# kheder-hassoun/Tf-IDF-Distributed-System

Hardware: AMD Instinct MI355X
Metric: docs indexed/sec + queries scored/sec (node) at 1/2/4/8 GPUs; % HBM roofline (higher is better)
Workload: dtype u8/u32 (integer inversion), f32 BM25 with f64 accumulation

## Files before the change

include/tfidf.h:

```cpp
#ifndef TFIDF_H
#define TFIDF_H

#include <stddef.h>
#include <stdint.h>

#ifdef __cplusplus
extern "C" {
#endif

#define TFIDF_OK 0
#define TFIDF_E_INVALID_ARG 1
#define TFIDF_E_HIP 2
#define TFIDF_E_OOM 3
#define TFIDF_E_UNSUPPORTED_INPUT 4
#define TFIDF_E_UNSUPPORTED_QUERY 5
#define TFIDF_E_CAPACITY 6
#define TFIDF_E_STATE 7
#define TFIDF_E_BUFFER 8
#define TFIDF_E_NO_DEVICE 9
#define TFIDF_E_QUERY_SYNTAX 10

#define TFIDF_STATS_SHARD 0
#define TFIDF_STATS_GLOBAL 1

// ... 6 lines not shown
typedef struct tfidf_config {
  float k1;
  float b;
  int32_t stats_mode;
  int32_t device;
  uint32_t vocab_capacity_log2;
  uint32_t max_token_len;
  int32_t inversion;
} tfidf_config;

typedef struct tfidf_index_stats {
  uint64_t num_docs;
  uint64_t doc_count;
  uint64_t sum_ttf;
  uint64_t num_terms;
  uint64_t nnz;
  uint64_t device_bytes;
  uint64_t long_docs;
  uint64_t text_bytes;
  uint64_t term_major;
  uint64_t pack_docs;
  uint64_t pack_retried;
  uint64_t unicode_docs;
  uint64_t long_chunked;
  uint64_t malformed_docs;
  uint64_t hash_seed;
  uint64_t hash_rebuilds;
  uint64_t coalesced_batches;
  uint64_t coalesced_queries;
  uint64_t unit_batches;
  uint64_t unit_count;
  uint64_t fused_queries;
  uint64_t unicode_wave_docs;
  uint64_t dead_docs;
  uint64_t dead_bytes;
  uint64_t compactions;
} tfidf_index_stats;

typedef struct tfidf_commit_timing {
  float ms_total;
  float ms_tokenize;
  float ms_long;
  float ms_df;
  float ms_blockscan;
  float ms_colscan;
  float ms_scatter;
  uint64_t text_bytes;
  uint64_t num_docs;
  uint64_t nnz;
} tfidf_commit_timing;

enum { TFIDF_MIRROR_NONE = 0, TFIDF_MIRROR_DELTA = 1, TFIDF_MIRROR_WHOLE = 2 };
typedef struct tfidf_host_profile {
  double ms_wall;
  double ms_counters;
  double ms_enqueued;
  double ms_synced;
  double ms_published;
  uint32_t stream_syncs;
  uint32_t col_rank_runs;
  uint32_t mirror_dict, mirror_df, mirror_crank;
  uint32_t dict_delta_entries, df_delta_entries;
  uint64_t bytes_dict, bytes_df, bytes_crank;
} tfidf_host_profile;

const char *tfidf_version(void);
const char *tfidf_last_error(void);
int tfidf_config_init(tfidf_config *cfg);

int tfidf_create(const tfidf_config *cfg, tfidf_index **out);
int tfidf_destroy(tfidf_index *ix);

int tfidf_add_docs(tfidf_index *ix, const uint8_t *utf8, const uint64_t *offsets, uint64_t n_docs,
                   const uint8_t *keys, const uint64_t *key_offsets);
int tfidf_clear(tfidf_index *ix);
int tfidf_add_docs_device(tfidf_index *ix, const void *d_utf8, const void *d_offsets, uint64_t n_docs,
                          uint64_t total_bytes);

int tfidf_commit(tfidf_index *ix);
int tfidf_commit_tokenized_docs(const tfidf_index *ix, uint64_t *docs, uint32_t *was_full);
int tfidf_commit_inverted_blocks(const tfidf_index *ix, uint32_t *first_block, uint32_t *n_blocks,
                                 uint32_t *remapped);
int tfidf_commit_inversion_shape(const tfidf_index *ix, uint32_t *slices, uint32_t *scan_parts);
int tfidf_commit_host_profile(const tfidf_index *ix, tfidf_host_profile *out);

int tfidf_delete_docs(tfidf_index *ix, const uint8_t *keys, const uint64_t *key_offsets, uint64_t n_keys,
                      uint64_t *n_deleted);
int tfidf_compact(tfidf_index *ix, uint64_t *bytes_reclaimed, float *ms_device);
int tfidf_set_compact_threshold(tfidf_index *ix, uint32_t dead_pct);
int tfidf_doc_text(tfidf_index *ix, uint64_t doc, uint8_t *buf, uint64_t cap, uint64_t *n_out);
int tfidf_set_hash_attempt(tfidf_index *ix, uint32_t attempt);

int tfidf_save(tfidf_index *ix, const char *path);
int tfidf_load(tfidf_index *ix, const char *path);
int tfidf_get_commit_timing(const tfidf_index *ix, tfidf_commit_timing *out);
int tfidf_stats(const tfidf_index *ix, tfidf_index_stats *out);

int tfidf_search(tfidf_index *ix, const uint8_t *q, uint64_t q_len, uint32_t k, uint32_t *doc_ids,
                 float *scores, uint64_t cap, uint64_t *n_out);
int tfidf_search_coalesced(tfidf_index *ix, const uint8_t *q, uint64_t q_len, uint32_t k, uint32_t *doc_ids,
                           float *scores, uint64_t cap, uint64_t *n_out, uint32_t wait_us);
int tfidf_search_batch(tfidf_index *ix, const uint8_t *q_utf8, const uint64_t *q_offsets, uint32_t n_q,
                       uint32_t k, uint32_t *doc_ids, float *scores, uint32_t *counts);
int tfidf_search_batch_all(tfidf_index *ix, const uint8_t *q_utf8, const uint64_t *q_offsets, uint32_t n_q,
                           uint32_t *doc_ids, float *scores, uint64_t cap, uint64_t *hit_offsets, uint64_t *n_out);
typedef struct tfidf_reader tfidf_reader;
int tfidf_reader_open(tfidf_index *ix, tfidf_reader **out);
int tfidf_reader_close(tfidf_reader *rd);
int tfidf_reader_info(const tfidf_reader *rd, uint64_t *generation, uint64_t *num_docs);
int tfidf_reader_search(tfidf_reader *rd, const uint8_t *q, uint64_t q_len, uint32_t k, uint32_t *doc_ids,
                        float *scores, uint64_t cap, uint64_t *n_out);
int tfidf_reader_search_batch_all(tfidf_reader *rd, const uint8_t *q_utf8, const uint64_t *q_offsets, uint32_t n_q,
                                  uint32_t *doc_ids, float *scores, uint64_t cap, uint64_t *hit_offsets,
                                  uint64_t *n_out);
int tfidf_reader_doc_key(const tfidf_reader *rd, uint64_t doc, uint8_t *buf, uint64_t cap, uint64_t *n_out);
int tfidf_reader_doc_text(const tfidf_reader *rd, uint64_t doc, uint8_t *buf, uint64_t cap, uint64_t *n_out);
int tfidf_reader_doc_keys(const tfidf_reader *rd, uint8_t *buf, uint64_t cap, uint64_t *offsets, uint64_t *n_bytes);
int tfidf_reader_matches(tfidf_reader *rd, const uint8_t *q, uint64_t q_len, const uint32_t *docs, uint64_t n_docs,
                         uint64_t *starts, uint32_t *lens, uint32_t *ordinals, uint64_t cap,
                         uint64_t *match_offsets, uint64_t *n_out, float *ms_device);
int tfidf_reader_snippets(tfidf_reader *rd, const uint8_t *q, uint64_t q_len, const uint32_t *docs, uint64_t n_docs,
                          uint32_t max_bytes, uint8_t *text, uint64_t text_cap, uint64_t *text_offsets,
                          uint64_t *doc_starts, uint64_t *starts, uint32_t *lens, uint32_t *ordinals, uint64_t m_cap,
                          uint64_t *match_offsets, uint64_t *n_text, uint64_t *n_matches, float *ms_device);
int tfidf_matches(tfidf_index *ix, const uint8_t *q, uint64_t q_len, const uint32_t *docs, uint64_t n_docs,
                  uint64_t *starts, uint32_t *lens, uint32_t *ordinals, uint64_t cap, uint64_t *match_offsets,
                  uint64_t *n_out, float *ms_device);
int tfidf_snippets(tfidf_index *ix, const uint8_t *q, uint64_t q_len, const uint32_t *docs, uint64_t n_docs,
                   uint32_t max_bytes, uint8_t *text, uint64_t text_cap, uint64_t *text_offsets, uint64_t *doc_starts,
                   uint64_t *starts, uint32_t *lens, uint32_t *ordinals, uint64_t m_cap, uint64_t *match_offsets,
                   uint64_t *n_text, uint64_t *n_matches, float *ms_device);
int tfidf_query_positive_terms(const uint8_t *q, uint64_t q_len, char *out, uint64_t cap, uint64_t *n_terms,
                               uint64_t *n_bytes);
int tfidf_reader_matches_batch(tfidf_reader *rd, const uint8_t *q_utf8, const uint64_t *q_offsets, uint32_t n_q,
                               const uint32_t *docs, const uint64_t *doc_offsets, uint64_t *starts, uint32_t *lens,
                               uint32_t *ordinals, uint64_t cap, uint64_t *match_offsets, uint64_t *n_out,
                               float *ms_device);
int tfidf_reader_snippets_batch(tfidf_reader *rd, const uint8_t *q_utf8, const uint64_t *q_offsets, uint32_t n_q,
                                const uint32_t *docs, const uint64_t *doc_offsets, uint32_t max_bytes, uint8_t *text,
                                uint64_t text_cap, uint64_t *text_offsets, uint64_t *doc_starts, uint64_t *starts,
                                uint32_t *lens, uint32_t *ordinals, uint64_t m_cap, uint64_t *match_offsets,
                                uint64_t *n_text, uint64_t *n_matches, float *ms_device);
int tfidf_matches_batch(tfidf_index *ix, const uint8_t *q_utf8, const uint64_t *q_offsets, uint32_t n_q,
                        const uint32_t *docs, const uint64_t *doc_offsets, uint64_t *starts, uint32_t *lens,
                        uint32_t *ordinals, uint64_t cap, uint64_t *match_offsets, uint64_t *n_out, float *ms_device);
int tfidf_snippets_batch(tfidf_index *ix, const uint8_t *q_utf8, const uint64_t *q_offsets, uint32_t n_q,
                         const uint32_t *docs, const uint64_t *doc_offsets, uint32_t max_bytes, uint8_t *text,
                         uint64_t text_cap, uint64_t *text_offsets, uint64_t *doc_starts, uint64_t *starts,
                         uint32_t *lens, uint32_t *ordinals, uint64_t m_cap, uint64_t *match_offsets,
                         uint64_t *n_text, uint64_t *n_matches, float *ms_device);
int tfidf_last_highlight_chunks(const tfidf_index *ix, uint64_t *item_chunks, uint64_t *row_chunks);
int tfidf_fuzzy_terms_batch(tfidf_index *ix, const uint8_t *t_utf8, const uint64_t *t_offsets, uint32_t n_terms,
                            uint32_t max_edits, uint32_t prefix_len, uint32_t max_out, uint64_t *cand_offsets,
                            uint64_t *n_within, uint64_t *term_offsets, uint8_t *terms, uint64_t terms_cap,
                            uint32_t *df, uint8_t *dist, uint64_t cand_cap, uint64_t *n_cands,
                            uint64_t *n_term_bytes, float *ms_device);
int tfidf_reader_fuzzy_terms_batch(tfidf_reader *rd, const uint8_t *t_utf8, const uint64_t *t_offsets,
                                   uint32_t n_terms, uint32_t max_edits, uint32_t prefix_len, uint32_t max_out,
                                   uint64_t *cand_offsets, uint64_t *n_within, uint64_t *term_offsets, uint8_t *terms,
                                   uint64_t terms_cap, uint32_t *df, uint8_t *dist, uint64_t cand_cap,
                                   uint64_t *n_cands, uint64_t *n_term_bytes, float *ms_device);
int tfidf_fuzzy_terms(tfidf_index *ix, const uint8_t *term, uint64_t len, uint32_t max_edits, uint32_t prefix_len,
                      uint32_t max_out, uint64_t *n_within, uint64_t *term_offsets, uint8_t *terms,
                      uint64_t terms_cap, uint32_t *df, uint8_t *dist, uint64_t cand_cap, uint64_t *n_cands,
                      uint64_t *n_term_bytes, float *ms_device);
int tfidf_reader_fuzzy_terms(tfidf_reader *rd, const uint8_t *term, uint64_t len, uint32_t max_edits,
// ... 318 lines not shown
```

tf-idf-distributed-system_amd/csrc/commit_plan.h:

```cpp
#pragma once

#include <stdint.h>
#include <stdlib.h>

#include <algorithm>
#include <vector>

namespace tfidf {

constexpr int kCommitKnobs = 11;
inline const char *const *commit_knob_names() {
  static const char *const names[kCommitKnobs] = {
      "TFIDF_NO_UNIWAVE", "TFIDF_NO_UNIFIRST",    "TFIDF_PACK_DOCS",  "TFIDF_NO_UCHUNK",       "TFIDF_TEST_PAIR_UNITS",
      "TFIDF_UW_FULL",    "TFIDF_TEST_WEAK_HASH", "TFIDF_DEBUG_STOP", "TFIDF_WAVE_WGS_PER_CU", "TFIDF_FULL_COMMIT",
      "TFIDF_TEST_G4_BITS"};
  return names;
}
constexpr int kKnobFullCommit = 9;

inline uint64_t knob_sig(const char *v) {
  if (!v) return 0;
  uint64_t h = 1469598103934665603ull;
  for (; *v; v++) h = (h ^ (uint8_t)*v) * 1099511628211ull;
  return h | (1ull << 63);
// ... 106 lines not shown
  p.base_after = (uint32_t)(N / kPlanBlockDocs);
  p.fold_first = inv.first_block;
  p.fold_end = std::max(p.base_after, inv.first_block);
  p.remap = inv.remap;
  p.from_rows = p.trusted && rows_knob && *rows_knob && !(rows_knob[0] == '0' && !rows_knob[1]);
  return p;
}

TFIDF_PLAN_HD uint32_t remap_base_value(const uint32_t *old_base, uint32_t old_bits, uint32_t old_base_col, uint32_t bit) {
  return (old_bits >> bit) & 1u ? old_base[remap_old_col(old_bits, old_base_col, bit)] : 0u;
}

inline uint64_t post_esc_keep(const std::vector<uint64_t> &sorted, uint64_t post_base) {
  return (uint64_t)(std::lower_bound(sorted.begin(), sorted.end(), post_base << 24) - sorted.begin());
}


constexpr uint32_t kSliceGroupDocs = 48;
constexpr uint32_t kSliceMinDocs = 192;
constexpr uint32_t kSliceWgsPerCu = 2;
constexpr uint32_t kScanPartCols = 16384;
constexpr uint32_t kScanPartAlign = 256;
constexpr uint32_t kSliceKnobMax = 256, kScanKnobMax = 64;
constexpr uint32_t kSortSpw = 4, kSortStreams = 64, kSortWgsPerCu = 2;

struct SlicePlan {
  uint32_t slices = 1;
  uint32_t slice_docs = (uint32_t)kPlanBlockDocs;
  uint32_t scan_parts = 1;
  uint32_t scan_width = 0;
  uint32_t sort_spw = 4;
};

inline SlicePlan slice_plan(uint32_t blocks, uint32_t R, uint64_t max_docs, uint32_t NC, uint32_t cus,
                            const char *slices_knob, const char *parts_knob) {
  SlicePlan p;
  if (blocks == 0 || R == 0) return p;
  while (p.sort_spw > 1 && (uint64_t)blocks * R * (kSortStreams / p.sort_spw) < (uint64_t)cus * kSortWgsPerCu)
    p.sort_spw /= 2;
  max_docs = std::min<uint64_t>(std::max<uint64_t>(max_docs, 1), kPlanBlockDocs);
  auto docs_for = [&](uint32_t s) {
    const uint64_t per = (max_docs + s - 1) / s;
    return (uint32_t)((per + kSliceGroupDocs - 1) / kSliceGroupDocs * kSliceGroupDocs);
  };
  if (slices_knob && *slices_knob) {
    p.slices = (uint32_t)std::max(1, std::min(atoi(slices_knob), (int)kSliceKnobMax));
    p.slice_docs = p.slices > 1 ? docs_for(p.slices) : (uint32_t)kPlanBlockDocs;
  } else {
    const uint64_t tiles = (uint64_t)blocks * R;
    const uint64_t by_grid = tiles >= cus ? 1 : (uint64_t)cus * kSliceWgsPerCu / tiles;
    const uint64_t by_docs = std::max<uint64_t>(1, max_docs / kSliceMinDocs);
    const uint32_t s = (uint32_t)std::min(by_grid, by_docs);
    if (s > 1) {
      p.slice_docs = docs_for(s);
      p.slices = (uint32_t)((max_docs + p.slice_docs - 1) / p.slice_docs);
      if (p.slices == 1) p.slice_docs = (uint32_t)kPlanBlockDocs;
    }
  }
  const uint32_t max_parts = std::max(1u, (uint32_t)(((uint64_t)NC + kScanPartCols - 1) / kScanPartCols));
  if (parts_knob && *parts_knob)
    p.scan_parts = (uint32_t)std::max(1, std::min(atoi(parts_knob), (int)kScanKnobMax));
  else
    p.scan_parts = std::min(max_parts, std::max(1u, cus / (2 * blocks)));
  if (p.scan_parts > 1) {
    const uint64_t per = std::max<uint64_t>(1, ((uint64_t)NC + p.scan_parts - 1) / p.scan_parts);
    p.scan_width = (uint32_t)((per + kScanPartAlign - 1) / kScanPartAlign * kScanPartAlign);
  }
  return p;
}

inline void slice_range(const SlicePlan &p, uint32_t i, uint64_t d0, uint64_t d1, uint64_t *lo, uint64_t *hi) {
  const uint64_t a = d0 + (uint64_t)i * p.slice_docs;
  *lo = std::min(a, d1);
  *hi = std::min(a + p.slice_docs, d1);
}
inline void scan_part_range(const SlicePlan &p, uint32_t j, uint32_t NC, uint64_t *lo, uint64_t *hi) {
  if (p.scan_parts <= 1) { *lo = 0; *hi = NC; return; }
  const uint64_t a = (uint64_t)j * p.scan_width;
  *lo = std::min<uint64_t>(a, NC);
  *hi = std::min<uint64_t>(a + p.scan_width, NC);
}


enum MirrorForm : uint32_t { kMirrorNone = 0, kMirrorDelta = 1, kMirrorWhole = 2 };

constexpr uint32_t kDictDeltaDiv = 32;
constexpr uint32_t kDictDeltaMin = 512;
inline uint32_t dict_delta_max(uint32_t C) { return std::min(C, std::max(C / kDictDeltaDiv, kDictDeltaMin)); }
constexpr uint32_t kDfDeltaCap = 1u << 12;
constexpr uint32_t kDfDeltaTry = 4;

struct DictDelta {
  uint64_t slot, lo, hi;
};
struct DfDelta {
  uint32_t slot, df;
};

struct MirrorPlan {
  bool delta = false;
  MirrorForm dict = kMirrorWhole, crank = kMirrorWhole, df = kMirrorWhole;
  uint32_t n_new = 0;
};

inline MirrorPlan mirror_plan(bool full, bool term_major, uint64_t kept_inv, bool mir_ok, uint32_t C, uint32_t NC,
                              uint32_t NC_inv, uint64_t new_nnz, uint32_t df_cap, const char *full_knob) {
  MirrorPlan p;
  const bool forced = full_knob && *full_knob && !(full_knob[0] == '0' && !full_knob[1]);
  if (full || term_major || kept_inv == 0 || !mir_ok || forced || NC < NC_inv) return p;
  p.delta = true;
  p.n_new = NC - NC_inv;
  if (p.n_new == 0) p.dict = p.crank = kMirrorNone;
  else if (p.n_new <= dict_delta_max(C)) p.dict = kMirrorDelta;
  if (new_nnz == 0) p.df = kMirrorNone;
  else if (new_nnz <= (uint64_t)df_cap * kDfDeltaTry) p.df = kMirrorDelta;
  return p;
}

inline bool df_slots_kept(const MirrorPlan &mp, uint64_t kept_inv, uint64_t N, bool remap, uint32_t NC, uint32_t NC_inv,
                          const char *always_knob) {
  const bool forced = always_knob && *always_knob && !(always_knob[0] == '0' && !always_knob[1]);
  return !forced && mp.delta && mp.df == kMirrorNone && mp.dict == kMirrorNone && kept_inv != 0 && kept_inv == N &&
         !remap && NC == NC_inv;
}

inline bool apply_dict_delta(uint64_t *h_dict, uint32_t C, const DictDelta *list, uint64_t n) {
  for (uint64_t i = 0; i < n; i++)
    if (list[i].slot >= C) return false;
  for (uint64_t i = 0; i < n; i++) {
    h_dict[list[i].slot] = list[i].lo;
    h_dict[(size_t)C + list[i].slot] = list[i].hi;
  }
  return true;
}
inline bool apply_df_delta(uint32_t *h_df, uint32_t C, const DfDelta *list, uint64_t n) {
  for (uint64_t i = 0; i < n; i++)
    if (list[i].slot >= C) return false;
  for (uint64_t i = 0; i < n; i++) h_df[list[i].slot] = list[i].df;
  return true;
}

}
```

tf-idf-distributed-system_amd/csrc/kernels_index.hip:

```cpp
#include <hip/hip_runtime.h>

#include <algorithm>

#include "dict_device.h"
#include "tfidf_common.h"
#include "unicode_scan.h"
#include "wave_ops.h"
#include "tfidf_internal.h"
#include "commit_plan.h"

namespace tfidf {


__device__ __forceinline__ void lds_barrier() { asm volatile("s_waitcnt lgkmcnt(0)\n\ts_barrier" ::: "memory"); }

__device__ __forceinline__ uint32_t block_excl_scan_256(uint32_t v, uint32_t *sh, uint32_t *total) {
  const uint32_t lane = threadIdx.x & 63, wid = threadIdx.x >> 6;
  uint32_t x = v;
#pragma unroll
  for (int o = 1; o < 64; o <<= 1) {
    uint32_t y = __shfl_up(x, o, 64);
    if (lane >= (uint32_t)o) x += y;
  }
  if (lane == 63) sh[wid] = x;
// ... 2008 lines not shown
      }
      const bool act = lo != 0;
      uint64_t mine = 0;
      if (act && (lo & kLoHashed)) {
        const uint64_t r = __hip_atomic_load(tpos + s, __ATOMIC_RELAXED, __HIP_MEMORY_SCOPE_AGENT);
        mine = dict_ref_word(s0 + dict_ref_off(r), dict_ref_len(r));
      }
      bool cl;
      uint32_t g = dict_find_or_insert(p.dict, p.cap_mask, act ? lo : 1, act ? hi : kKeyValid, act, &mine, &cl);
      if (act && (lo & kLoHashed) && !cl && g != kInvalidSlot) dict_verify(p, g, mine, d);
      if (act) {
        if (g == kInvalidSlot) { set_err(p.err, kErrCapacity, d); g = 0; }
        gsl[s] = g;
        atomicAdd(&sm.rcnt[g >> p.range_shift], 1u);
        my_nu++;
      }
    }
    atomicAdd(&sm.nu, my_nu);
    __syncthreads();
    if (tid == 0) {
      uint32_t run = 0;
      for (uint32_t r = 0; r < p.n_ranges; r++) {
        const uint32_t c = sm.rcnt[r];
        sm.rcur[r] = run;
        run += c;
        p.rsplit[(uint64_t)d * p.n_ranges + r] = run;
        sm.rcnt[r] = 0;
      }
      const uint32_t len = sm.len;
      p.doc_len[d] = len;
      p.doc_nuniq[d] = sm.nu;
      p.doc_norm[d] = (uint8_t)int_to_byte4(len);
      my_doc_count += len > 0;
      my_ttf += len;
      my_nnz += sm.nu;
    }
    __syncthreads();
    const uint64_t base = csr_row_base(p.offsets, src);
    for (uint32_t s = tid; s < T; s += 256) {
      if (__hip_atomic_load(keys + 2 * (size_t)s, __ATOMIC_RELAXED, __HIP_MEMORY_SCOPE_AGENT) == 0) continue;
      const uint32_t g = gsl[s];
      const uint32_t pos = atomicAdd(&sm.rcur[g >> p.range_shift], 1u);
      csr_put(p, base + pos, g, __hip_atomic_load(cnt + s, __ATOMIC_RELAXED, __HIP_MEMORY_SCOPE_AGENT), d);
    }
    __syncthreads();
    if (tid == 0) { sm.len = 0; sm.flags = 0; sm.nu = 0; }
    __syncthreads();
  }
  if (tid == 0) {
    atomicAdd(&p.stats[0], my_doc_count);
    atomicAdd(&p.stats[1], my_ttf);
    atomicAdd(&p.stats[2], my_nnz);
  }
}


__device__ __forceinline__ void doc_segment(const PostingParams &p, uint64_t d, uint32_t r, uint64_t *base,
                                            uint32_t *lo, uint32_t *hi) {
  const uint64_t src = p.live_map ? p.live_map[d] : d;
  *base = csr_row_base(p.offsets, src);
  *lo = r ? p.rsplit[d * p.n_ranges + r - 1] : 0;
  *hi = p.rsplit[d * p.n_ranges + r];
}

#ifndef TFIDF_DF_QUADS
#define TFIDF_DF_QUADS 4
#endif
#ifndef TFIDF_PART_QUADS
#define TFIDF_PART_QUADS 3
#endif
constexpr int kDfQuads = TFIDF_DF_QUADS;
constexpr int kPartQuads = TFIDF_PART_QUADS;
static_assert(kDfQuads >= 1 && kDfQuads <= 4 && kPartQuads >= 1 && kPartQuads <= 4, "quads per group");

typedef uint32_t csr_quad_t __attribute__((ext_vector_type(4), aligned(4)));

template <int Q>
struct InvQuads {
  uint64_t at[Q];
  uint32_t n[Q];
};

template <int Q>
__device__ __forceinline__ InvQuads<Q> inv_quads(const PostingParams &p, uint64_t dd, uint64_t d1, uint32_t r) {
  const uint32_t lane = threadIdx.x & 63;
  const uint64_t d = dd + lane;
  uint64_t at = 0;
  uint32_t n = 0;
  if (lane < (uint32_t)(4 * Q) && d < d1) {
    const uint64_t src = p.live_map ? p.live_map[d] : d;
    const uint32_t lo = r ? p.rsplit[d * p.n_ranges + r - 1] : 0;
    at = csr_row_base(p.offsets, src) + lo;
    n = p.rsplit[d * p.n_ranges + r] - lo;
  }
  InvQuads<Q> g;
#pragma unroll
  for (int q = 0; q < Q; q++) {
    const int from = 4 * q + (int)(lane >> 4);
    g.at[q] = ((uint64_t)(uint32_t)__shfl((int)(uint32_t)(at >> 32), from, 64) << 32) |
              (uint32_t)__shfl((int)(uint32_t)at, from, 64);
    g.n[q] = (uint32_t)__shfl((int)n, from, 64);
  }
  return g;
}

template <int Q>
__device__ __forceinline__ uint32_t inv_maxn(const InvQuads<Q> &g) {
  uint32_t m = 0;
#pragma unroll
  for (int q = 0; q < Q; q++) m = max(m, g.n[q]);
  return m;
}

template <int Q>
__device__ __forceinline__ void inv_load(const PostingParams &p, const InvQuads<Q> &g, uint32_t off, uint32_t *c) {
  const uint32_t e0 = off + 4 * (threadIdx.x & 15);
#pragma unroll
  for (int q = 0; q < Q; q++) {
    const uint32_t n = g.n[q];
    csr_quad_t v = {0u, 0u, 0u, 0u};
    if (e0 < n) v = *reinterpret_cast<const csr_quad_t *>(p.csr + g.at[q] + e0);
    c[4 * q] = v.x;
    c[4 * q + 1] = e0 + 1 < n ? v.y : 0u;
    c[4 * q + 2] = e0 + 2 < n ? v.z : 0u;
    c[4 * q + 3] = e0 + 3 < n ? v.w : 0u;
  }
}

__device__ __forceinline__ bool tile_of(uint32_t w, uint32_t n_blocks, uint32_t R, uint32_t *b, uint32_t *r) {
  const uint32_t g = w / (8 * R), rem = w - g * 8 * R;
  *r = rem >> 3;
  *b = g * 8 + (rem & 7);
  return *b < n_blocks;
}
static uint32_t tiles_grid(uint32_t n_blocks, uint32_t R) { return (n_blocks + 7) / 8 * 8 * R; }

template <bool SLICED>
__global__ void __launch_bounds__(1024) k_df_partial(PostingParams p) {
  extern __shared__ uint32_t hist[];
  uint32_t b, r, slice = 0;
  if (!tile_of(blockIdx.x, (p.n_blocks - p.first_block) * (SLICED ? p.slices : 1u), p.n_ranges, &b, &r)) return;
  if (SLICED) {
    slice = b % p.slices;
    b /= p.slices;
  }
  b += p.first_block;
  const uint32_t RS = 1u << p.range_shift;
  uint64_t d0 = (uint64_t)b * kBlockDocs;
  uint64_t d1 = d0 + kBlockDocs < p.n_docs ? d0 + kBlockDocs : p.n_docs;
  if (SLICED) {
    d0 += (uint64_t)slice * p.slice_docs;
    if (d0 >= d1) return;
    d1 = d0 + p.slice_docs < d1 ? d0 + p.slice_docs : d1;
  }
  for (uint32_t i = threadIdx.x; i < RS / 2; i += blockDim.x) hist[i] = 0;
  __syncthreads();
  const uint32_t nw = blockDim.x >> 6;
  const uint32_t wid = (uint32_t)__builtin_amdgcn_readfirstlane((int)(threadIdx.x >> 6));
  const uint32_t rmask = RS - 1;
  constexpr int Q = kDfQuads, E = 4 * Q;
  const uint64_t step = (uint64_t)nw * E;
  uint64_t dd = d0 + (uint64_t)wid * E;
  InvQuads<Q> cur = inv_quads<Q>(p, dd, d1, r);
  uint32_t c[E];
  inv_load<Q>(p, cur, 0, c);
  auto count = [&](uint32_t e) __attribute__((always_inline)) {
    const uint32_t sl = e & rmask;
    atomicAdd(&hist[sl >> 1], 1u << ((sl & 1u) << 4));
  };
  while (dd < d1) {
    const uint64_t dn = dd + step;
    const InvQuads<Q> nxt = inv_quads<Q>(p, dn, d1, r);
    uint32_t cn[E];
    inv_load<Q>(p, nxt, 0, cn);
#pragma unroll
    for (int j = 0; j < E; j++)
      if (c[j]) count(c[j]);
    const uint32_t maxn = inv_maxn<Q>(cur);
    for (uint32_t off = 64; __any(off < maxn); off += 64) {
      inv_load<Q>(p, cur, off, c);
#pragma unroll
      for (int j = 0; j < E; j++)
        if (c[j]) count(c[j]);
    }
    cur = nxt;
#pragma unroll
    for (int j = 0; j < E; j++) c[j] = cn[j];
    dd = dn;
  }
  __syncthreads();
  uint32_t *out = p.blk + (size_t)b * p.NC;
  const uint32_t w0 = (r << p.range_shift) >> 5;
  for (uint32_t w = threadIdx.x; w < (RS >> 5); w += blockDim.x) {
    const uint2 e = p.crank[w0 + w];
    uint32_t bits = e.x, col = e.y;
    while (bits) {
      const uint32_t sl = 32 * w + (uint32_t)__builtin_ctz(bits);
      bits &= bits - 1;
      const uint32_t n = (hist[sl >> 1] >> ((sl & 1u) << 4)) & 0xFFFFu;
      if (!SLICED) out[col] = n;
      else if (n) atomicAdd(&out[col], n);
      col++;
    }
  }
}

__device__ __forceinline__ uint32_t df_from_kept_rows(const PostingParams &p, uint64_t t) {
  const bool last = t + 1 == p.NC;
  const uint32_t *own = p.blk + t, *nxt = own + (last ? 0 : 1);
  uint32_t lo = 0, hi = 0, b = 0;
  for (; b + 8 <= p.first_block; b += 8) {
    uint32_t x[8], y[8];
#pragma unroll
    for (int j = 0; j < 8; j++) {
      x[j] = own[(size_t)(b + j) * p.NC];
      y[j] = nxt[(size_t)(b + j) * p.NC];
    }
#pragma unroll
    for (int j = 0; j < 8; j++) { lo += x[j]; hi += y[j]; }
  }
  for (; b < p.first_block; b++) {
    lo += own[(size_t)b * p.NC];
    hi += nxt[(size_t)b * p.NC];
  }
  return (last ? (uint32_t)(p.bbase[p.first_block] - p.bbase[0]) : hi) - lo;
}

template <bool PARTS>
__global__ void __launch_bounds__(256) k_df_sum(PostingParams p) {
  __shared__ uint32_t psum[2][4];
  const uint64_t t = (uint64_t)blockIdx.x * blockDim.x + threadIdx.x;
  const bool in = t < p.NC;
  if (!PARTS && !in) return;
  const uint32_t lane = threadIdx.x & 63, wid = threadIdx.x >> 6;
  const uint32_t base = in && p.first_block ? p.df_base[t] : 0u;
  uint32_t run = base;
  if (p.df_from_rows && in && p.first_block) run = df_from_kept_rows(p, t);
  uint32_t full = 0, tail = 0;
  if (!PARTS) {
    for (uint32_t b = p.first_block; b < p.df_fold_end; b++) full += p.blk[(size_t)b * p.NC + t];
    for (uint32_t b = p.df_fold_end; b < p.n_blocks; b++) tail += p.blk[(size_t)b * p.NC + t];
  } else {
    for (uint32_t b = p.first_block; b < p.n_blocks; b++) {
      const uint32_t v = in ? p.blk[(size_t)b * p.NC + t] : 0u;
      if (b < p.df_fold_end) full += v;
      else tail += v;
      uint32_t *ps = psum[(b - p.first_block) & 1u];
      const uint32_t w = wave_sum(v);
      if (lane == 0) ps[wid] = w;
      __syncthreads();
      if (threadIdx.x == 0)
        p.part_tot[(size_t)(b - p.first_block) * gridDim.x + blockIdx.x] = ps[0] + ps[1] + ps[2] + ps[3];
    }
    if (!in) return;
  }
  p.blk[(size_t)p.n_blocks * p.NC + t] = run + full + tail;
  if (!p.first_block || p.df_fold_end > p.first_block) p.df_base[t] = base + full;
}

__global__ void __launch_bounds__(256) k_blk_remap(PostingParams p, const uint32_t *blk_old, const uint32_t *df_old,
                                                   const uint2 *crank_inv, uint32_t NC_inv) {
  const uint32_t w = blockIdx.x * blockDim.x + threadIdx.x, b = blockIdx.y;
  if (w >= (p.C >> 5)) return;
  const uint2 e = p.crank[w], o = crank_inv[w];
  if (b == p.first_block) {
    uint32_t bits = e.x, col = e.y;
    while (bits) {
      const uint32_t bit = (uint32_t)__builtin_ctz(bits);
      bits &= bits - 1;
      p.df_base[col++] = remap_base_value(df_old, o.x, o.y, bit);
    }
    return;
// ... 275 lines not shown
    const uint32_t s0 = (r << p.range_shift) + k * BS;
    const uint2 *kw = wk + (k - k0) * (BS / 32);
    const uint32_t c0 = kw[0].y, c1 = kw[BS / 32].y;
    if (c0 == c1) continue;
    for (uint32_t i = threadIdx.x; i < BS; i += blockDim.x) {
      const uint2 e = kw[i >> 5];
      const uint32_t bit = 1u << (i & 31u);
      if (e.x & bit) cur[i] = row[e.y + __popc(e.x & (bit - 1u))];
    }
    const uint32_t lo = row[c0];
    const uint32_t hi = c1 < p.NC ? row[c1] : btot;
    const bool staged = hi - lo <= kSortStage;
    __syncthreads();
    constexpr int U = 8;
    for (uint32_t e0 = lo; e0 < hi; e0 += U * blockDim.x) {
      uint32_t x[U], nrm[U];
#pragma unroll
      for (int u = 0; u < U; u++) {
        const uint32_t e = e0 + u * blockDim.x + threadIdx.x;
        x[u] = e < hi ? p.post_tmp[bb + e] : 0u;
      }
#pragma unroll
      for (int u = 0; u < U; u++) {
        const uint32_t e = e0 + u * blockDim.x + threadIdx.x;
        nrm[u] = e < hi ? bnorm[x[u] & (kBlockDocs - 1)] : 0u;
      }
#pragma unroll
      for (int u = 0; u < U; u++) {
        const uint32_t e = e0 + u * blockDim.x + threadIdx.x;
        if (__all(e >= hi)) break;
        const bool in = e < hi;
        const uint32_t sl = in ? (x[u] >> 13) & (kSubSlots - 1) : kSubSlots;
        const uint32_t pos = atomicAdd(&cur[sl], 1u);
        const uint32_t doc = d0 + (x[u] & (kBlockDocs - 1));
        uint32_t tf = x[u] >> kTmpTfShift;
        if (in && tf == kTmpTfEsc) tf = csr_tf_of(p, doc, r, s0 + sl);
        if (in) {
          const uint32_t w = post_word(x[u] & (kBlockDocs - 1), tf, nrm[u]);
          if (staged) ostage[pos - lo] = w;
          else p.post[bb + pos] = w;
          if (tf >= kPostTfEsc) {
            const uint32_t at = atomicAdd(p.post_esc_count, 1u);
            if (at < p.post_esc_cap) p.post_esc[at] = ((bb + pos) << 24) | tf;
          }
        }
      }
    }
    __syncthreads();
    if (staged)
      for (uint32_t i = threadIdx.x; i < hi - lo; i += blockDim.x) p.post[bb + lo + i] = ostage[i];
    __syncthreads();
  }
}

__global__ void __launch_bounds__(1024) k_block_scan(PostingParams p) {
  __shared__ uint64_t wsum[16];
  const uint32_t B = p.n_blocks;
  const uint32_t tid = threadIdx.x, lane = tid & 63, wid = tid >> 6;
  uint64_t carry = p.first_block ? p.bbase[p.first_block] : 0ull;
  for (uint32_t i0 = p.first_block; i0 < B; i0 += 1024) {
    const uint32_t i = i0 + tid;
    const uint64_t v = i < B ? p.bbase[i + 1] : 0ull;
    uint64_t x = v;
#pragma unroll
    for (int o = 1; o < 64; o <<= 1) {
      const uint64_t y = __shfl_up(x, o, 64);
      if (lane >= (uint32_t)o) x += y;
    }
    if (lane == 63) wsum[wid] = x;
    __syncthreads();
    uint64_t base = carry, all = 0;
    for (uint32_t w = 0; w < 16; w++) {
      const uint64_t s = wsum[w];
      if (w < wid) base += s;
      all += s;
    }
    __syncthreads();
    if (i < B) p.bbase[i + 1] = base + x;
    carry += all;
  }
  if (tid == 0 && p.first_block == 0) p.bbase[0] = 0;
}

__global__ void __launch_bounds__(256) k_verify_deferred(BuildParams p) {
  const uint32_t n = min(*p.verify_count, p.verify_cap);
  const uint64_t *ref = p.dict + 2 * ((size_t)p.cap_mask + 1);
  for (uint32_t i = blockIdx.x * blockDim.x + threadIdx.x; i < n; i += gridDim.x * blockDim.x) {
    const uint32_t slot = (uint32_t)p.verify_defer[2 * (size_t)i];
    const uint64_t mine = p.verify_defer[2 * (size_t)i + 1], r = ref[slot];
    if (r == mine) continue;
    if (r == 0 || !uc_same_term(p.text + dict_ref_off(r), dict_ref_len(r), p.text + dict_ref_off(mine),
                                dict_ref_len(mine)))
      set_build_err(p.err, kErrCollision, 0);
  }
}


hipError_t launch_verify_deferred(const BuildParams &p, hipStream_t s) {
  hipLaunchKernelGGL(k_verify_deferred, dim3(64), dim3(256), 0, s, p);
  return hipGetLastError();
}

#ifndef TFIDF_G4_BITS
#define TFIDF_G4_BITS 21
#endif
static bool use_g4(const BuildParams &p) {
  uint32_t bits = TFIDF_G4_BITS;
  if (const char *e = knob("TFIDF_TEST_G4_BITS")) bits = (uint32_t)std::max(4, std::min(atoi(e), 32));
  return (uint64_t)p.cap_mask + 1 >= (1ull << bits);
}

__global__ void __launch_bounds__(256) k_doc_range(uint32_t *list, uint32_t *count, uint32_t first, uint32_t n) {
  const uint32_t i = blockIdx.x * 256u + threadIdx.x;
  if (i < n) list[i] = first + i;
  if (i == 0) *count = n;
}
hipError_t launch_doc_range(uint32_t *list, uint32_t *count, uint32_t first, uint32_t n, hipStream_t s) {
  hipLaunchKernelGGL(k_doc_range, dim3((n + 255) / 256 ? (n + 255) / 256 : 1), dim3(256), 0, s, list, count, first, n);
  return hipGetLastError();
}

hipError_t launch_tokenize_wave(const BuildParams &p, int grid, hipStream_t s) {
  const bool g4 = use_g4(p);
  if (p.pack > 1) {
    if (g4) hipLaunchKernelGGL((k_tokenize_wave<true, true>), dim3(grid), dim3(64), 0, s, p);
    else hipLaunchKernelGGL((k_tokenize_wave<true, false>), dim3(grid), dim3(64), 0, s, p);
  } else {
    if (g4) hipLaunchKernelGGL((k_tokenize_wave<false, true>), dim3(grid), dim3(64), 0, s, p);
    else hipLaunchKernelGGL((k_tokenize_wave<false, false>), dim3(grid), dim3(64), 0, s, p);
  }
  return hipGetLastError();
}
hipError_t launch_tokenize_wave_uni(const BuildParams &p, int grid, hipStream_t s) {
  const bool g4 = use_g4(p);
  if (g4) hipLaunchKernelGGL((k_tokenize_wave<false, true, true>), dim3(grid), dim3(64), 0, s, p);
  else hipLaunchKernelGGL((k_tokenize_wave<false, false, true>), dim3(grid), dim3(64), 0, s, p);
  return hipGetLastError();
}
hipError_t launch_tokenize_chunks(const BuildParams &p, int grid, hipStream_t s) {
  hipLaunchKernelGGL(k_tokenize_chunk<false>, dim3(grid), dim3(64), 0, s, p);
  return hipGetLastError();
}
hipError_t launch_tokenize_chunks_uni(const BuildParams &p, int grid, hipStream_t s) {
  hipLaunchKernelGGL(k_tokenize_chunk<true>, dim3(grid), dim3(64), 0, s, p);
  return hipGetLastError();
}
hipError_t launch_long_rows(const BuildParams &p, uint32_t n_docs, hipStream_t s) {
  static std::atomic<uint64_t> big{0};
  allow_dyn_lds((const void *)k_long_rows, 4 * kLrWin, big);
  const uint32_t C = p.cap_mask + 1;
  hipLaunchKernelGGL(k_long_rows, dim3(n_docs), dim3(kLrThreads), (C < kLrWin ? C : kLrWin) * 4, s, p);
  return hipGetLastError();
}
hipError_t launch_tokenize_long(const BuildParams &p, int grid, hipStream_t s) {
  hipLaunchKernelGGL(k_tokenize_long, dim3(grid), dim3(256), 0, s, p);
  return hipGetLastError();
}
static void allow_big_lds() {
  static std::atomic<uint64_t> done{0}, done_sliced{0};
  allow_dyn_lds((const void *)k_df_partial<false>, 2 << kRangeBits, done);
  allow_dyn_lds((const void *)k_df_partial<true>, 2 << kRangeBits, done_sliced);
}

static_assert(kSliceGroupDocs % (4 * kDfQuads) == 0 && kSliceGroupDocs % (4 * kPartQuads) == 0,
              "a slice is a whole number of the loaders' document groups");
static_assert(kScanPartAlign == 256 && kScanPartCols == 16384, "k_df_sum's workgroup, k_row_scan's round");

__global__ void __launch_bounds__(256) k_inv_zero(uint32_t *rows, uint64_t n_rows, uint32_t *aux, uint64_t n_aux) {
  const uint64_t stride = (uint64_t)gridDim.x * blockDim.x;
  for (uint64_t i = (uint64_t)blockIdx.x * blockDim.x + threadIdx.x; i < n_rows + n_aux; i += stride) {
    if (i < n_rows) rows[i] = 0;
    else aux[i - n_rows] = 0;
  }
}
hipError_t launch_inv_zero(const PostingParams &p, hipStream_t s) {
  const uint64_t nb = p.n_blocks - p.first_block;
  if (nb == 0 || p.slices <= 1) return hipSuccess;
  const uint64_t n_rows = nb * p.NC;
  const uint64_t n_cur = nb * p.n_ranges * kPartStreams;
  if (p.scan_parts > 1 && p.part_tot != p.slice_cur + n_cur) return hipErrorInvalidValue;
  const uint64_t n = n_rows + n_cur;
  const uint32_t grid = (uint32_t)std::max<uint64_t>(1, std::min<uint64_t>((n + 1023) / 1024, 1024));
  hipLaunchKernelGGL(k_inv_zero, dim3(grid), dim3(256), 0, s, p.blk + (size_t)p.first_block * p.NC, n_rows, p.slice_cur,
                     n_cur);
  return hipGetLastError();
}

hipError_t launch_df_partial(const PostingParams &p, hipStream_t s) {
  allow_big_lds();
  const size_t lds = (size_t)2 << p.range_shift;
  if (p.n_blocks == p.first_block) return hipSuccess;
  const uint32_t nb = p.n_blocks - p.first_block;
  if (p.slices > 1)
    hipLaunchKernelGGL(k_df_partial<true>, dim3(tiles_grid(nb * p.slices, p.n_ranges)), dim3(1024), lds, s, p);
  else
    hipLaunchKernelGGL(k_df_partial<false>, dim3(tiles_grid(nb, p.n_ranges)), dim3(1024), lds, s, p);
  return hipGetLastError();
}
hipError_t launch_df_sum(const PostingParams &p, hipStream_t s) {
  if (p.NC == 0) return hipSuccess;
  if (!p.df_base || p.df_fold_end < p.first_block || p.df_fold_end > p.n_blocks) return hipErrorInvalidValue;
  if (p.scan_parts > 1 && p.n_blocks != p.first_block)
    hipLaunchKernelGGL(k_df_sum<true>, dim3((p.NC + 255) / 256), dim3(256), 0, s, p);
  else
    hipLaunchKernelGGL(k_df_sum<false>, dim3((p.NC + 255) / 256), dim3(256), 0, s, p);
  return hipGetLastError();
}
hipError_t launch_row_scan(const PostingParams &p, hipStream_t s) {
  if (p.n_blocks == p.first_block) return hipSuccess;
  const uint32_t nb = p.n_blocks - p.first_block;
  if (p.scan_parts > 1) hipLaunchKernelGGL(k_row_scan_parts, dim3(nb * p.scan_parts), dim3(1024), 0, s, p);
  else hipLaunchKernelGGL(k_row_scan, dim3(nb), dim3(1024), 0, s, p);
  return hipGetLastError();
}
hipError_t launch_blk_remap(const PostingParams &p, const uint32_t *blk_old, const uint32_t *df_old,
                            const uint2 *crank_inv, uint32_t NC_inv, hipStream_t s) {
  if (!p.first_block || !(p.C >> 5)) return hipSuccess;
  if (!df_old || !p.df_base || df_old == p.df_base) return hipErrorInvalidValue;
  hipLaunchKernelGGL(k_blk_remap, dim3(((p.C >> 5) + 255) / 256, p.first_block + 1), dim3(256), 0, s, p, blk_old, df_old,
                     crank_inv, NC_inv);
  return hipGetLastError();
}
__global__ void __launch_bounds__(256) k_count_nonzero(const uint64_t *a, uint32_t n, unsigned long long *out) {
  uint32_t c = 0;
  for (uint32_t i = blockIdx.x * blockDim.x + threadIdx.x; i < n; i += gridDim.x * blockDim.x) {
    const uint64_t m = __ballot(a[i] != 0);
    c += (uint32_t)__popcll(m);
  }
  if ((threadIdx.x & 63) == 0 && c) atomicAdd(out, (unsigned long long)c);
}
hipError_t launch_count_nonzero(const uint64_t *a, uint32_t n, unsigned long long *out, hipStream_t s) {
  const uint32_t grid = std::max(1u, std::min((n + 255) / 256, 2048u));
  hipLaunchKernelGGL(k_count_nonzero, dim3(grid), dim3(256), 0, s, a, n, out);
  return hipGetLastError();
}
__global__ void __launch_bounds__(256) k_crank_bits(const uint64_t *lo, uint32_t C, uint2 *crank) {
  const uint32_t s0 = (blockIdx.x * blockDim.x + threadIdx.x) & ~63u, lane = threadIdx.x & 63;
  if (s0 >= C) return;
  const uint64_t m = __ballot(lo[s0 + lane] != 0);
  if (lane < 2) crank[(s0 >> 5) + lane] = make_uint2(lane ? (uint32_t)(m >> 32) : (uint32_t)m, 0u);
}
__global__ void __launch_bounds__(1024) k_crank_scan(uint2 *crank, uint32_t W, unsigned long long *n_cols) {
  __shared__ uint32_t wsum[16];
  __shared__ uint32_t carry_sh;
  const uint32_t tid = threadIdx.x, lane = tid & 63, wid = tid >> 6;
  if (tid == 0) carry_sh = 0;
  __syncthreads();
  for (uint32_t t0 = 0; t0 < W; t0 += 16384) {
    const uint32_t i0 = t0 + tid * 16;
    uint32_t v[16], tot = 0;
#pragma unroll
    for (int q = 0; q < 16; q++) {
      v[q] = i0 + q < W ? (uint32_t)__popc(crank[i0 + q].x) : 0u;
      tot += v[q];
    }
    const uint32_t x = wave_incl_add(tot);
    if (lane == 63) wsum[wid] = x;
    __syncthreads();
    uint32_t base = carry_sh, all = 0;
    for (uint32_t w = 0; w < 16; w++) {
      const uint32_t sw = wsum[w];
      if (w < wid) base += sw;
      all += sw;
    }
    base += x - tot;
    __syncthreads();
    if (tid == 0) carry_sh += all;
#pragma unroll
    for (int q = 0; q < 16; q++) {
      if (i0 + q < W) crank[i0 + q].y = base;
      base += v[q];
    }
    __syncthreads();
  }
  if (tid == 0) {
    crank[W] = make_uint2(0u, carry_sh);
    *n_cols = carry_sh;
  }
}
// ... 79 lines not shown
```

tf-idf-distributed-system_amd/csrc/tfidf_capi.hip:

```cpp
#include <hip/hip_runtime.h>

#include <math.h>
#include <stdarg.h>
#include <stdio.h>
#include <stdlib.h>
#include <string.h>

#include <algorithm>
#include <atomic>
#include <chrono>
#include <condition_variable>
#include <functional>
#include <memory>
#include <mutex>
#include <string>
#include <thread>
#include <unordered_map>
#include <unordered_set>
#include <vector>

#include "../../include/tfidf.h"
#include "analysis.h"
#include "commit_plan.h"
#include "compact_plan.h"
// ... 299 lines not shown
  bool q_timing = true;
  DevMem q_in, q_out, cand, cand_n, out_doc, out_score, hits, hits_n, hits_c, hits_s, hits_P, ovf;
  DevMem hl_in, hl_cnt, hl_m, hl_s, hl_o;
  DevMem fz_in, fz_hs, fz_c, fz_tmp;
  DevMem fz_o;
  DevMem ph_in, ph_s, ph_o, ph_tmp;
  DevMem ml_in, ml_c, ml_tmp;
  DevMem wc_bits, wc_cnt, wc_out, wc_len;
  DevMem rx_tab;
  PinnedVec<uint32_t> q_host, q_res, q_cand_h;
  std::vector<uint64_t> q_merge;
  std::vector<uint32_t> q_units;
  uint32_t *res_doc = nullptr, *res_n = nullptr;
  float *res_score = nullptr;
  explicit SearchCtx(int d)
      : dev(d), q_in(d), q_out(d), cand(d), cand_n(d), out_doc(d), out_score(d), hits(d), hits_n(d), hits_c(d),
        hits_s(d), hits_P(d), ovf(d), hl_in(d), hl_cnt(d), hl_m(d), hl_s(d), hl_o(d), fz_in(d), fz_hs(d), fz_c(d),
        fz_tmp(d), fz_o(d), ph_in(d), ph_s(d), ph_o(d), ph_tmp(d), ml_in(d), ml_c(d), ml_tmp(d), wc_bits(d),
        wc_cnt(d), wc_out(d), wc_len(d), rx_tab(d) {}
  int init() {
    DeviceGuard g(dev);
    if (hipStreamCreateWithFlags(&own, hipStreamNonBlocking) != hipSuccess ||
        hipStreamCreateWithFlags(&side, hipStreamNonBlocking) != hipSuccess)
      return fail(TFIDF_E_HIP, "hipStreamCreate failed");
    for (int i = 0; i < QEV_N; i++) hipEventCreate(&ev[i]);
    for (int i = 0; i < 2; i++) hipEventCreateWithFlags(&q_ev[i], hipEventDisableTiming);
    hipEventCreateWithFlags(&q_in_ev, hipEventDisableTiming);
    return TFIDF_OK;
  }
  ~SearchCtx() {
    DeviceGuard g(dev);
    if (own) hipStreamSynchronize(own);
    if (side) hipStreamSynchronize(side);
    for (int i = 0; i < QEV_N; i++) if (ev[i]) hipEventDestroy(ev[i]);
    for (int i = 0; i < 2; i++) if (q_ev[i]) hipEventDestroy(q_ev[i]);
    if (q_in_ev) hipEventDestroy(q_in_ev);
    if (side) hipStreamDestroy(side);
    if (own) hipStreamDestroy(own);
  }
};

struct tfidf_index {
  tfidf_config cfg;
  std::mutex mu;
  hipStream_t stream = nullptr;
  hipStream_t own_stream = nullptr;
  hipStream_t user_stream = nullptr;
  hipEvent_t ev[EV_N];
  hipStream_t copy_stream = nullptr;
  hipEvent_t mir_ev[3];
  int num_cus = 256;

  std::mutex snap_mu;
  std::shared_ptr<Snapshot> cur, spare;
  uint64_t generation = 0;

  std::mutex ctx_mu;
  std::vector<std::unique_ptr<SearchCtx>> ctx_free;
  std::atomic<bool> q_timing{true};
  std::mutex ms_mu;
  float last_ms_scoring = 0, last_ms_total = 0;
  uint64_t last_hl_item_chunks = 0, last_hl_row_chunks = 0;
  uint64_t last_fz_scan_chunks = 0, last_fz_cand_chunks = 0;
  uint64_t last_ph_candidates = 0, last_ph_row_chunks = 0;
  uint64_t last_mlt_entries = 0, last_mlt_chunks = 0;
  uint64_t last_wc_scan_chunks = 0, last_wc_matches = 0, last_wc_union_chunks = 0;
  uint64_t last_rx_scan_chunks = 0, last_rx_matches = 0, last_rx_union_chunks = 0, last_rx_table_bytes = 0;

  std::shared_ptr<DevMem> text, offsets;
  void *stage[2] = {nullptr, nullptr};
  hipEvent_t stage_ev[2] = {nullptr, nullptr};
  uint64_t text_bytes = 0, n_staged = 0;
  std::vector<uint64_t> h_offsets{0};
  KeyTable keys;
  std::vector<uint8_t> staged_live;
  std::unordered_map<std::string, uint64_t> key_to_staged;
  uint64_t n_dead = 0;
  uint64_t dead_bytes = 0;
  uint64_t corpus_epoch = 0;
  uint64_t last_tok_docs = 0;
  uint32_t last_tok_full = 1;
  uint32_t last_inv_first = 0, last_inv_blocks = 0, last_inv_remap = 0;
  uint32_t last_inv_slices = 1, last_inv_scan_parts = 1;
  tfidf_host_profile prof{};
  std::chrono::steady_clock::time_point prof_t0;
  uint64_t next_ord = 0;
  uint32_t compact_pct = 0;
  uint64_t compactions = 0;

  uint32_t cap_log2 = 18;
  DevBuf d_live_map;
  DevBuf long_list, uni_list, counters, post_tmp;
  DevBuf retry_list;
  DevBuf new_list;
  DevBuf mir_dict_list, mir_df_list;
  DevBuf inv_aux;
  PinnedVec<DictDelta> h_dict_delta;
  PinnedVec<DfDelta> h_df_delta;
  DevBuf bad_list;
  uint64_t hash_seed = 0;
  uint32_t hash_rebuilds = 0;
  bool uni_first = false;
  uint32_t hash_floor = 0;
  uint32_t collision_doc = 0;
  mutable std::mutex cq_mu;
  std::condition_variable cq_cv;
  std::vector<struct CoalesceReq *> cq;
  bool cq_leader = false;
  size_t cq_max = kCoalesceMaxDefault;
  uint64_t cq_batches = 0, cq_queries = 0;
  std::atomic<uint64_t> unit_batches{0}, unit_count{0}, fused_queries{0};
  DevBuf verify_defer, lt_pos;
  DevBuf tvals, term_tmp, term_esc;
  DevBuf lt_keys, lt_cnt, lt_g;
  DevBuf pairs, pair_ub, chunk_list, chunk_docs, chunk_fail, uchunk;
  PinnedVec<uint32_t> ldocs_h, pre_h;
  PinnedVec<uint64_t> hctr_h;
  uint32_t lt_log2 = 0, lt_wgs = 64;
  tfidf_commit_timing timing{};

  DevBuf canon_of_slot;
  uint64_t n_canon = 0;
  DevBuf sent_slot, vcounts, vnu, vt_table, vt_sum, vt_rslot, gdf_dev;
  uint64_t n_sent = 0;
  std::shared_ptr<StatsView> view_spare;
};

int StatsView::wait_gdf() {
  std::lock_guard<std::mutex> lk(gdf_mu);
  if (gdf_pending) {
    HIP_TRY(hipEventSynchronize(gdf_ev));
    gdf_pending = false;
  }
  return TFIDF_OK;
}

static std::shared_ptr<Snapshot> current(tfidf_index *ix, std::shared_ptr<StatsView> *v = nullptr) {
  std::lock_guard<std::mutex> lk(ix->snap_mu);
  if (v) *v = ix->cur ? ix->cur->stats : nullptr;
  return ix->cur;
}
static std::shared_ptr<Snapshot> current(const tfidf_index *ix, std::shared_ptr<StatsView> *v = nullptr) {
  return current(const_cast<tfidf_index *>(ix), v);
}

struct CtxLease {
  tfidf_index *ix;
  std::unique_ptr<SearchCtx> c;
  int rc = TFIDF_OK;
  explicit CtxLease(tfidf_index *x) : ix(x) {
    {
      std::lock_guard<std::mutex> lk(ix->ctx_mu);
      if (!ix->ctx_free.empty()) {
        c = std::move(ix->ctx_free.back());
        ix->ctx_free.pop_back();
      }
    }
    if (!c) {
      c.reset(new SearchCtx(ix->cfg.device));
      rc = c->init();
    }
    c->q_timing = ix->q_timing.load();
  }
  ~CtxLease() {
    if (!c || rc) return;
    {
      DeviceGuard g(ix->cfg.device);
      const hipStream_t st = stream();
      if (hipStreamQuery(st) != hipSuccess) hipStreamSynchronize(st);
      if (c->side && hipStreamQuery(c->side) != hipSuccess) hipStreamSynchronize(c->side);
    }
    std::lock_guard<std::mutex> lk(ix->ctx_mu);
    ix->ctx_free.push_back(std::move(c));
  }
  hipStream_t stream() const { return ix->user_stream ? ix->user_stream : c->own; }
};


extern "C" const char *tfidf_version(void) { return "libtfidf 0.1.0 (gfx950)"; }
extern "C" const char *tfidf_last_error(void) { return g_err.c_str(); }

extern "C" int tfidf_config_init(tfidf_config *cfg) {
  if (!cfg) return fail(TFIDF_E_INVALID_ARG, "cfg is NULL");
  cfg->k1 = 1.2f;
  cfg->b = 0.75f;
  cfg->stats_mode = TFIDF_STATS_SHARD;
  cfg->device = 0;
  cfg->vocab_capacity_log2 = 18;
  cfg->max_token_len = 255;
  cfg->inversion = TFIDF_INVERSION_AUTO;
  return TFIDF_OK;
}

extern "C" int tfidf_create(const tfidf_config *cfg, tfidf_index **out) {
  if (!cfg || !out) return fail(TFIDF_E_INVALID_ARG, "NULL argument");
  if (cfg->max_token_len != 255) return fail(TFIDF_E_INVALID_ARG, "only max_token_len = 255 is supported");
  uint32_t lg = cfg->vocab_capacity_log2 ? cfg->vocab_capacity_log2 : 18;
  if (lg < 10 || lg > 26) return fail(TFIDF_E_INVALID_ARG, "vocab_capacity_log2 must be in [10, 26]");
  if (lg > kMaxBlockCapLog2 && cfg->inversion == TFIDF_INVERSION_BLOCK)
    return fail(TFIDF_E_INVALID_ARG, "block-major inversion supports vocab_capacity_log2 <= %u", kMaxBlockCapLog2);
  if (!(std::isfinite(cfg->k1) && cfg->k1 >= 0.f))
    return fail(TFIDF_E_INVALID_ARG, "k1 must be finite and >= 0 (got %g)", (double)cfg->k1);
  if (!(cfg->b >= 0.f && cfg->b <= 1.f)) return fail(TFIDF_E_INVALID_ARG, "b must be in [0, 1] (got %g)", (double)cfg->b);
  int ndev = 0;
  if (hipGetDeviceCount(&ndev) != hipSuccess || ndev == 0) return fail(TFIDF_E_NO_DEVICE, "no HIP device");
  if (cfg->device < 0 || cfg->device >= ndev) return fail(TFIDF_E_NO_DEVICE, "device %d out of range", cfg->device);
  DeviceGuard g(cfg->device);
  tfidf_index *ix = new tfidf_index();
  ix->cfg = *cfg;
  ix->cfg.vocab_capacity_log2 = lg;
  ix->cap_log2 = lg;
  hipDeviceProp_t prop;
  if (hipGetDeviceProperties(&prop, cfg->device) == hipSuccess) ix->num_cus = prop.multiProcessorCount;
  if (hipStreamCreateWithFlags(&ix->own_stream, hipStreamNonBlocking) != hipSuccess) {
    delete ix;
    return fail(TFIDF_E_HIP, "hipStreamCreate failed");
  }
  ix->stream = ix->own_stream;
  if (const char *cm = knob("TFIDF_COALESCE_MAX")) ix->cq_max = std::max(1, atoi(cm));
  if (hipStreamCreateWithFlags(&ix->copy_stream, hipStreamNonBlocking) != hipSuccess) {
    hipStreamDestroy(ix->own_stream);
    delete ix;
    return fail(TFIDF_E_HIP, "hipStreamCreate failed");
  }
  for (int i = 0; i < EV_N; i++) hipEventCreate(&ix->ev[i]);
  for (int i = 0; i < 2; i++) hipEventCreateWithFlags(&ix->stage_ev[i], hipEventDisableTiming);
  for (int i = 0; i < 3; i++) hipEventCreateWithFlags(&ix->mir_ev[i], hipEventDisableTiming);
  ix->text = std::make_shared<DevMem>(cfg->device);
  ix->offsets = std::make_shared<DevMem>(cfg->device);
  hipError_t e = ix->offsets->reserve(64);
  if (e != hipSuccess) { delete ix; return fail(TFIDF_E_OOM, "hipMalloc offsets"); }
  uint64_t zero = 0;
  hipMemcpy(ix->offsets->p, &zero, 8, hipMemcpyHostToDevice);
  *out = ix;
  return TFIDF_OK;
}

extern "C" int tfidf_destroy(tfidf_index *ix) {
  if (!ix) return TFIDF_OK;
  DeviceGuard g(ix->cfg.device);
  hipStreamSynchronize(ix->stream);
  hipStreamSynchronize(ix->copy_stream);
  ix->cur.reset();
  ix->spare.reset();
  ix->ctx_free.clear();
  ix->text.reset();
  ix->offsets.reset();
  DevBuf *bufs[] = {&ix->d_live_map, &ix->long_list, &ix->uni_list, &ix->counters, &ix->retry_list, &ix->new_list, &ix->bad_list,
                    &ix->mir_dict_list, &ix->mir_df_list, &ix->inv_aux,
                    &ix->post_tmp, &ix->lt_keys, &ix->lt_cnt, &ix->lt_g, &ix->lt_pos, &ix->verify_defer, &ix->pairs,
                    &ix->pair_ub, &ix->chunk_list, &ix->chunk_docs, &ix->chunk_fail, &ix->uchunk, &ix->canon_of_slot,
                    &ix->tvals, &ix->term_tmp, &ix->term_esc, &ix->sent_slot, &ix->vcounts, &ix->vnu, &ix->vt_table,
                    &ix->vt_sum, &ix->vt_rslot, &ix->gdf_dev};
  for (DevBuf *b : bufs) b->release();
  for (int i = 0; i < EV_N; i++) hipEventDestroy(ix->ev[i]);
  for (int i = 0; i < 2; i++) {
    if (ix->stage[i]) hipHostFree(ix->stage[i]);
    hipEventDestroy(ix->stage_ev[i]);
  }
  for (int i = 0; i < 3; i++) hipEventDestroy(ix->mir_ev[i]);
  hipStreamSynchronize(ix->own_stream);
  hipStreamDestroy(ix->copy_stream);
  hipStreamDestroy(ix->own_stream);
  delete ix;
  return TFIDF_OK;
}

static int grow_shared(tfidf_index *ix, std::shared_ptr<DevMem> *buf, uint64_t need, uint64_t keep, bool zero) {
  if (need <= (*buf)->bytes) return TFIDF_OK;
  uint64_t cap = (*buf)->bytes ? (*buf)->bytes : (1ull << 20);
  while (cap < need) cap = cap + cap / 2 + (1ull << 20);
  auto nb = std::make_shared<DevMem>(ix->cfg.device);
  HIP_TRY(nb->reserve(cap));
  if (zero) HIP_TRY(hipMemsetAsync(nb->p, 0, cap, ix->stream));
  if ((*buf)->p && keep) HIP_TRY(hipMemcpyAsync(nb->p, (*buf)->p, keep, hipMemcpyDeviceToDevice, ix->stream));
  HIP_TRY(hipStreamSynchronize(ix->stream));
  *buf = std::move(nb);
  return TFIDF_OK;
}

static int grow_text(tfidf_index *ix, uint64_t extra) {
  return grow_shared(ix, &ix->text, ix->text_bytes + extra + 128, ix->text_bytes, true);
}

static int grow_offsets(tfidf_index *ix, uint64_t extra_docs) {
  return grow_shared(ix, &ix->offsets, (ix->n_staged + extra_docs + 1) * 8, (ix->n_staged + 1) * 8, false);
}

static int grow_keep(tfidf_index *ix, DevMem *buf, uint64_t need, uint64_t keep) {
  if (!keep || !buf->p) {
    HIP_TRY(buf->reserve(need));
    return TFIDF_OK;
  }
  if (need <= buf->bytes) return TFIDF_OK;
  uint64_t cap = buf->bytes;
  while (cap < need) cap = cap + cap / 2 + (1ull << 20);
  DevMem nb(buf->dev);
  if (nb.reserve(cap) != hipSuccess) {
    hipGetLastError();
    HIP_TRY(nb.reserve(need));
  }
  HIP_TRY(hipMemcpyAsync(nb.p, buf->p, std::min<uint64_t>(keep, buf->bytes), hipMemcpyDeviceToDevice, ix->stream));
  HIP_TRY(hipStreamSynchronize(ix->stream));
  std::swap(buf->p, nb.p);
  std::swap(buf->bytes, nb.bytes);
  return TFIDF_OK;
}

static bool kill_staged(tfidf_index *ix, uint64_t st) {
  if (!ix->staged_live[st]) return false;
  ix->staged_live[st] = 0;
  ix->n_dead++;
  ix->corpus_epoch++;
  ix->dead_bytes += ix->h_offsets[st + 1] - ix->h_offsets[st];
  return true;
}

static void register_key(tfidf_index *ix, const uint8_t *k, uint64_t n, bool synth) {
  const uint64_t idx = ix->n_staged;
  KeyChunk &c = ix->keys.tail(idx, ix->next_ord++);
  if (!synth) {
    std::string key((const char *)k, n);
    auto it = ix->key_to_staged.find(key);
    if (it != ix->key_to_staged.end()) {
      kill_staged(ix, it->second);
      it->second = idx;
    } else {
      ix->key_to_staged.emplace(std::move(key), idx);
    }
    c.arena.append((const char *)k, n);
  }
  c.off.push_back(c.arena.size());
// ... 633 lines not shown
  bp.verify_defer = ix->verify_defer.as<uint64_t>();
  bp.verify_count = reinterpret_cast<uint32_t *>(ctr + 11);
  bp.verify_cap = kVerifyCap;
  bp.csr = S.csr.as<uint32_t>();
  bp.csr_esc = S.csr_esc.as<uint64_t>();
  bp.esc_count = reinterpret_cast<uint32_t *>(ctr + 9);
  bp.esc_cap = esc_cap;
  bp.doc_len = S.doc_len.as<uint32_t>();
  bp.doc_nuniq = S.doc_nuniq.as<uint32_t>();
  bp.doc_norm = S.doc_norm.as<uint8_t>();
  bp.rsplit = S.rsplit.as<uint32_t>();
  bp.long_list = ix->long_list.as<uint32_t>();
  bp.long_count = reinterpret_cast<uint32_t *>(ctr + 4);
  bp.uni_list = ix->uni_list.as<uint32_t>();
  bp.uni_count = reinterpret_cast<uint32_t *>(ctr + 6);
  bp.uni_wave_count = reinterpret_cast<uint32_t *>(ctr + 13);
  bp.bad_list = ix->bad_list.as<uint32_t>();
  bp.bad_count = reinterpret_cast<uint32_t *>(ctr + 8);
  bp.stats = reinterpret_cast<unsigned long long *>(ctr);
  bp.err = reinterpret_cast<uint32_t *>(ctr + 3);
  if (const char *ds = knob("TFIDF_DEBUG_STOP")) bp.debug_stop = (uint32_t)atoi(ds);
  if (const char *uf = knob("TFIDF_UW_FULL")) bp.debug_uw_full = (uint32_t)atoi(uf);
  bp.pack = pack;
  bp.retry_list = pack > 1 ? ix->retry_list.as<uint32_t>() : nullptr;
  bp.retry_count = reinterpret_cast<uint32_t *>(ctr + 5);
  S.pack_docs = pack;
  S.pack_retried = kept.pack_retried;

  HIP_TRY(hipEventRecord(ix->ev[EV_START], s));
  if (N > d_first) {
    const uint64_t n_new = N - d_first;
    const uint64_t units = (n_new + pack - 1) / pack;
    uint64_t wpc = kWaveWGsPerCU;
    if (const char *e = knob("TFIDF_WAVE_WGS_PER_CU")) wpc = (uint64_t)std::max(1, atoi(e));
    const uint64_t grid = std::min<uint64_t>(units, (uint64_t)ix->num_cus * wpc);
    bp.first_doc = d_first;
    if (d_first && pack == 1 && !uni_first) {
      HIP_TRY(ix->new_list.reserve(n_new * 4 + 8));
      uint32_t *nl = ix->new_list.as<uint32_t>();
      HIP_TRY(launch_doc_range(nl + 1, nl, (uint32_t)d_first, (uint32_t)n_new, s));
      BuildParams np = bp;
      np.doc_list = nl + 1;
      np.doc_list_count = nl;
      HIP_TRY(launch_tokenize_wave(np, (int)grid, s));
    } else if (!uni_first) HIP_TRY(launch_tokenize_wave(bp, (int)grid, s));
    if (pack > 1 && !bp.debug_stop) {
      uint32_t n_retry = 0;
      HIP_TRY(hipMemcpyAsync(&n_retry, ctr + 5, 4, hipMemcpyDeviceToHost, s));
      HIP_TRY(commit_sync(ix, s));
      S.pack_retried = kept.pack_retried + n_retry;
      if (n_retry) {
        BuildParams rp = bp;
        rp.pack = 1;
        rp.doc_list = bp.retry_list;
        rp.doc_list_count = bp.retry_count;
        const uint64_t rgrid = std::min<uint64_t>(n_retry, (uint64_t)ix->num_cus * kWaveWGsPerCU);
        HIP_TRY(launch_tokenize_wave(rp, (int)rgrid, s));
      }
    }
    if (bp.debug_stop < 10 && uni_on)
      HIP_TRY(launch_tokenize_wave_uni(bp, (int)std::min<uint64_t>((N + 63) / 64, (uint64_t)ix->num_cus * kWaveWGsPerCU), s));
    if (!bp.debug_stop || bp.debug_stop >= 10)
      HIP_TRY(launch_tokenize_uwave(bp, (int)std::min<uint64_t>(N, (uint64_t)ix->num_cus * kUwaveWGsPerCU), s));
  }
  HIP_TRY(hipEventRecord(ix->ev[EV_TOK], s));
  if (bp.debug_stop) {
    HIP_TRY(commit_sync(ix, s));
    ix->timing = tfidf_commit_timing{};
    ix->timing.ms_tokenize = ev_ms(ix, EV_START, EV_TOK);
    ix->timing.ms_total = ix->timing.ms_tokenize;
    ix->timing.text_bytes = ix->text_bytes;
    ix->timing.num_docs = N;
    return kRcNoPublish;
  }
  auto col_rank = [&]() -> int {
    if (!S.term_major && !keep_rank) {
      HIP_TRY(launch_col_rank(S.dict.as<uint64_t>(), C, S.crank.as<uint2>(),
                              reinterpret_cast<unsigned long long *>(ctr + 7), s));
      ix->prof.col_rank_runs++;
    }
    return TFIDF_OK;
  };
  if (int rc = col_rank()) return rc;
  HIP_TRY(ix->hctr_h.resize(14));
  uint64_t *hctr = ix->hctr_h.data();
  HIP_TRY(hipMemcpyAsync(hctr, ctr, 14 * sizeof(uint64_t), hipMemcpyDeviceToHost, s));
  HIP_TRY(commit_sync(ix, s));
  ix->prof.ms_counters = prof_ms(ix);
  const uint32_t n_long = (uint32_t)hctr[4], n_uni = (uint32_t)hctr[6];
  S.long_chunked = kept.long_chunked;
  S.long_docs = kept.long_docs + n_long;
  S.unicode_docs = kept.unicode_docs + n_uni + (uint32_t)hctr[13];
  S.unicode_wave_docs = kept.unicode_wave_docs + (uint32_t)hctr[13];
  ix->uni_first = pack == 1 && (uint64_t)S.unicode_docs * 2 > N;
  if (n_long) {
    HIP_TRY(hipEventRecord(ix->ev[EV_L0], s));
    PinnedVec<uint32_t> &ldocs = ix->ldocs_h;
    HIP_TRY(ldocs.resize(n_long));
    HIP_TRY(hipMemcpyAsync(ldocs.data(), ix->long_list.p, (size_t)n_long * 4, hipMemcpyDeviceToHost, s));
    HIP_TRY(commit_sync(ix, s));
    const uint32_t wlog = std::min<uint32_t>(ix->cap_log2, kLrWinBits);
    const uint32_t bsh = std::max<uint32_t>(wlog, ix->cap_log2 > 6 ? ix->cap_log2 - 6 : 0);
    const uint32_t nb = 1u << (ix->cap_log2 - bsh);
    uint64_t unit_max = std::max<uint64_t>(1, kPairBudget / ((uint64_t)kPairWords * 4));
    if (const char *e = knob("TFIDF_TEST_PAIR_UNITS")) unit_max = std::max(1, atoi(e));
    std::vector<uint32_t> pre;
    std::vector<uint64_t> gpre, gdoc;
    uint64_t acc = 0, max_units = 0;
    for (uint64_t i = 0; i < n_long; i++) {
      const uint64_t st = S.live_map.empty() ? ldocs[i] : S.live_map[ldocs[i]];
      const uint64_t L = ix->h_offsets[st + 1] - ix->h_offsets[st];
      const uint64_t units = (L + kLongCoreBytes - 1) / kLongCoreBytes;
      if (i == 0 || acc + units > unit_max) {
        if (i) { pre.push_back((uint32_t)acc); max_units = std::max(max_units, acc); }
        gpre.push_back(pre.size());
        gdoc.push_back(i);
        acc = 0;
      }
      pre.push_back((uint32_t)acc);
      acc += units;
      if (acc >= 0xFFFFFFFFull) return fail(TFIDF_E_CAPACITY, "too many document chunks");
    }
    pre.push_back((uint32_t)acc);
    max_units = std::max(max_units, acc);
    gdoc.push_back(n_long);
    HIP_TRY(ix->pairs.reserve(max_units * kPairWords * 4));
    HIP_TRY(ix->pair_ub.reserve(max_units * (nb + 1) * 4));
    HIP_TRY(ix->chunk_list.reserve(pre.size() * 4 + 8));
    HIP_TRY(ix->chunk_docs.reserve((size_t)n_long * 4));
    HIP_TRY(ix->chunk_fail.reserve((size_t)n_long * 4));
    HIP_TRY(ix->uchunk.reserve(max_units * 4 + 16));
    HIP_TRY(ix->pre_h.resize(pre.size()));
    memcpy(ix->pre_h.data(), pre.data(), pre.size() * 4);
    HIP_TRY(hipMemcpyAsync(ix->chunk_list.p, ix->pre_h.data(), pre.size() * 4, hipMemcpyHostToDevice, s));
    HIP_TRY(hipMemcpyAsync(ix->chunk_docs.p, ix->long_list.p, (size_t)n_long * 4, hipMemcpyDeviceToDevice, s));
    HIP_TRY(hipMemsetAsync(ix->chunk_fail.p, 0, (size_t)n_long * 4, s));
    HIP_TRY(hipMemsetAsync(bp.long_count, 0, 4, s));
    for (size_t gi = 0; gi < gpre.size(); gi++) {
      const uint64_t g0 = gdoc[gi], n = gdoc[gi + 1] - g0;
      BuildParams cp = bp;
      cp.chunk_pre = ix->chunk_list.as<uint32_t>() + gpre[gi];
      cp.n_group_docs = (uint32_t)n;
      cp.n_chunks = pre[gpre[gi] + n];
      cp.chunk_docs = ix->chunk_docs.as<uint32_t>() + g0;
      cp.chunk_fail = ix->chunk_fail.as<uint32_t>() + g0;
      cp.pairs = ix->pairs.as<uint32_t>();
      cp.pair_ub = ix->pair_ub.as<uint32_t>();
      cp.pair_bshift = bsh;
      cp.pair_nb = nb;
      const bool uch = !knob("TFIDF_NO_UCHUNK");
      cp.uchunk_count = uch ? ix->uchunk.as<uint32_t>() : nullptr;
      cp.uchunk_list = uch ? ix->uchunk.as<uint32_t>() + 4 : nullptr;
      if (uch) HIP_TRY(hipMemsetAsync(ix->uchunk.p, 0, (size_t)(cp.n_chunks + 4) * 4, s));
      const uint64_t grid = std::min<uint64_t>(cp.n_chunks, (uint64_t)ix->num_cus * kWaveWGsPerCU);
      HIP_TRY(launch_tokenize_chunks(cp, (int)grid, s));
      const char *nouw = knob("TFIDF_NO_UNIWAVE");
      if (uch && !(nouw && *nouw && *nouw != '0')) HIP_TRY(launch_tokenize_chunks_uni(cp, (int)grid, s));
      if (uch)
        HIP_TRY(launch_tokenize_uchunk(cp, (int)std::min<uint64_t>(cp.n_chunks, (uint64_t)ix->num_cus * kUchunkWGsPerCU), s));
      HIP_TRY(launch_long_rows(cp, (uint32_t)n, s));
    }
    uint32_t n_fb = 0;
    HIP_TRY(hipMemcpyAsync(&n_fb, bp.long_count, 4, hipMemcpyDeviceToHost, s));
    HIP_TRY(commit_sync(ix, s));
    S.long_chunked = kept.long_chunked + n_long - n_fb;
    if (n_fb) {
      uint32_t lg = ix->cap_log2 + 1;
// ... 2 lines not shown
      uint32_t need = 10;
      while (need < 22 && (1ull << need) < maxlen + 2) need++;
      lg = std::min(lg, need);
      ix->lt_log2 = lg;
      const uint64_t per_wg = 24ull << lg;
      const uint64_t by_budget = std::max<uint64_t>(ix->lt_wgs, kLongScratchBudget / per_wg);
      const uint32_t wgs = (uint32_t)std::min<uint64_t>({(uint64_t)n_fb, (uint64_t)ix->num_cus * 2, by_budget});
      HIP_TRY(ix->lt_keys.reserve((size_t)wgs * 2 * (1ull << lg) * 8));
      HIP_TRY(ix->lt_cnt.reserve((size_t)wgs * (1ull << lg) * 4));
      HIP_TRY(ix->lt_pos.reserve((size_t)wgs * (1ull << lg) * 8));
      HIP_TRY(ix->lt_g.reserve((size_t)wgs * (1ull << lg) * 4));
      bp.lt_keys = ix->lt_keys.as<uint64_t>();
      bp.lt_cnt = ix->lt_cnt.as<uint32_t>();
      bp.lt_pos = ix->lt_pos.as<uint64_t>();
      bp.lt_g = ix->lt_g.as<uint32_t>();
      bp.lt_slots_log2 = lg;
      HIP_TRY(launch_tokenize_long(bp, (int)wgs, s));
    }
    HIP_TRY(hipEventRecord(ix->ev[EV_LONG], s));
    if (int rc = col_rank()) return rc;
    HIP_TRY(hipMemcpyAsync(hctr, ctr, 10 * sizeof(uint64_t), hipMemcpyDeviceToHost, s));
    HIP_TRY(commit_sync(ix, s));
  }
  const uint32_t err = (uint32_t)(hctr[3] & 0xFFFFFFFFu), err_doc = (uint32_t)(hctr[3] >> 32);
  if (err & kErrCollision) { ix->collision_doc = err_doc; return kRcCollision; }
  if (err) {
    if (err & kErrCapacity)
      return fail(TFIDF_E_CAPACITY, "vocabulary exceeds 2^%u dictionary slots (raise vocab_capacity_log2)",
                  ix->cap_log2);
    return fail(TFIDF_E_UNSUPPORTED_INPUT, "index build error flags 0x%x (doc %u)", err, err_doc);
  }
  S.doc_count = kept.doc_count + hctr[0];
  S.sum_ttf = kept.sum_ttf + hctr[1];
  S.nnz = kept.nnz + hctr[2];
  S.NC = S.term_major ? 0u : keep_rank ? S.NC_inv : (uint32_t)hctr[7];
  if (!S.stats || S.stats.use_count() > 1) S.stats = std::make_shared<StatsView>(ix->cfg.device);
  {
    StatsView &V = *S.stats;
    if (int rc = V.wait_gdf()) return rc;
    V.global = false;
    V.gdf.clear();
    V.doc_count = S.doc_count;
    V.sum_ttf = S.sum_ttf;
    if (int rc = upload_cache(ix->cfg, V, s, false)) return rc;
  }
  const InversionPlan inv = inversion_plan(plan.full, S.term_major, kept_inv, N, S.NC, S.NC_inv,
                                           knob("TFIDF_FULL_INVERSION"));
  const uint32_t first_block = inv.first_block;
  const DfBasePlan dbp = df_base_plan(inv, S.term_major, N, knob("TFIDF_DF_FROM_ROWS"));
  uint32_t df_cap = kDfDeltaCap;
  if (const char *e = knob("TFIDF_TEST_DF_DELTA_CAP")) df_cap = (uint32_t)std::max(1, std::min(atoi(e), (int)kDfDeltaCap));
  const MirrorPlan mp = mirror_plan(plan.full, S.term_major, kept_inv, mir_was_ok, C, S.NC, S.NC_inv, hctr[2], df_cap,
                                    knob("TFIDF_FULL_MIRROR"));
  const bool keep_sdf = !plan.full && !S.term_major &&
                        df_slots_kept(mp, kept_inv, N, inv.remap, S.NC, S.NC_inv, knob("TFIDF_DF_SLOTS_ALWAYS"));
  const bool dict_delta = mp.dict == kMirrorDelta, df_delta = mp.df == kMirrorDelta;
  const bool dict_whole = mp.dict == kMirrorWhole, df_whole = mp.df == kMirrorWhole, crank_whole = mp.crank == kMirrorWhole;
  if (dict_delta) {
    HIP_TRY(ix->mir_dict_list.reserve((size_t)dict_delta_max(C) * sizeof(DictDelta)));
    HIP_TRY(ix->h_dict_delta.resize(dict_delta_max(C)));
  }
  if (df_delta) {
    HIP_TRY(ix->mir_df_list.reserve((size_t)kDfDeltaCap * sizeof(DfDelta)));
    HIP_TRY(ix->h_df_delta.resize(kDfDeltaCap));
  }
  const uint64_t kept_post = first_block ? S.h_bbase[first_block] : 0;
  const uint64_t kept_pe = first_block ? post_esc_keep(S.h_post_esc, kept_post) : 0;
  ix->last_inv_first = first_block;
  ix->last_inv_blocks = S.n_blocks;
  ix->last_inv_remap = inv.remap ? 1u : 0u;
  SlicePlan sp;
  if (!S.term_major) {
    const uint32_t inv_blocks = S.n_blocks - first_block;
    const uint64_t max_docs = inv_blocks == 0 ? 0 : inv_blocks > 1 ? kBlockDocs : N - (uint64_t)first_block * kBlockDocs;
    sp = slice_plan(inv_blocks, S.R, max_docs, S.NC, (uint32_t)ix->num_cus, knob("TFIDF_TEST_INV_SLICES"),
                    knob("TFIDF_TEST_SCAN_PARTS"));
    if (sp.slices > 1 || sp.scan_parts > 1)
      HIP_TRY(ix->inv_aux.reserve_slack(((uint64_t)inv_blocks * S.R * 64 * (sp.slices > 1) +
                                         (uint64_t)inv_blocks * ((S.NC + kScanPartAlign - 1) / kScanPartAlign) *
                                             (sp.scan_parts > 1)) * 4));
  }
  ix->last_inv_slices = sp.slices;
  ix->last_inv_scan_parts = sp.scan_parts;
  const uint32_t *blk_old = nullptr, *df_old = nullptr;
  if (!S.term_major) {
    const uint64_t blk_need = (uint64_t)(S.n_blocks + 1) * S.NC * 4 + 16;
    const uint64_t base_need = (uint64_t)S.NC * 4 + 16;
    if (inv.remap) {
      HIP_TRY(S.blk_alt.reserve(blk_need + blk_need / 8));
      std::swap(S.blk.p, S.blk_alt.p);
      std::swap(S.blk.bytes, S.blk_alt.bytes);
      blk_old = S.blk_alt.as<uint32_t>();
      HIP_TRY(S.df_base_alt.reserve(base_need + base_need / 8));
      std::swap(S.df_base.p, S.df_base_alt.p);
      std::swap(S.df_base.bytes, S.df_base_alt.bytes);
      df_old = S.df_base_alt.as<uint32_t>();
    } else {
      if (int rc = grow_keep(ix, &S.blk, blk_need, (uint64_t)first_block * S.NC * 4)) return rc;
      if (int rc = grow_keep(ix, &S.df_base, base_need + base_need / 8, dbp.trusted ? (uint64_t)S.NC * 4 : 0)) return rc;
    }
    if (int rc = grow_keep(ix, &S.bbase, (uint64_t)(S.n_blocks + 2) * 8, first_block ? (uint64_t)(first_block + 1) * 8 : 0))
      return rc;
  }
  {
    const EscAppend ea = esc_append_bounds(kept_esc, (uint32_t)hctr[9], esc_cap);
    if (ea.overflow) return fail(TFIDF_E_CAPACITY, "CSR escape list overflow");
    const uint64_t n_esc = ea.first + ea.count;
    S.h_esc.resize(n_esc);
    if (ea.count) {
      HIP_TRY(hipMemcpyAsync(S.h_esc.data() + ea.first, S.csr_esc.as<uint64_t>() + ea.first, ea.count * 8,
                             hipMemcpyDeviceToHost, s));
      HIP_TRY(commit_sync(ix, s));
      esc_merge(&S.h_esc, ea.first);
      HIP_TRY(hipMemcpyAsync(S.csr_esc.p, S.h_esc.data(), n_esc * 8, hipMemcpyHostToDevice, s));
      HIP_TRY(commit_sync(ix, s));
    }
  }
  if (S.nnz >= 0xFFFFFFFFull) return fail(TFIDF_E_CAPACITY, "more than 2^32 postings per shard");
  if (int rc = grow_keep(ix, &S.post, S.nnz * (S.term_major ? 8 : 4) + 8, kept_post * 4)) return rc;
  HIP_TRY(ix->post_tmp.reserve_slack(S.nnz * (S.term_major ? 8 : 4) + 8));
  const uint64_t post_esc_cap = row_cap / kPostTfEsc + 64;
  if (!S.term_major)
    if (int rc = grow_keep(ix, &S.post_esc, post_esc_cap * 8, kept_pe * 8)) return rc;
  if (kept_pe) HIP_TRY(hipMemsetD32Async((hipDeviceptr_t)(ctr + 10), (int)(uint32_t)kept_pe, 1, s));

  HIP_TRY(S.h_dict.resize((size_t)2 * C));
  HIP_TRY(S.h_df.resize(C));
  static const bool mirror_main = knob("TFIDF_MIRROR_MAIN") != nullptr;
  const bool mirror_side = (!mirror_main && s == ix->own_stream) || (size_t)2 * C * 8 >= (32u << 20);
  const bool side_work = mirror_side && !(mp.delta && N == d_first);
  if (side_work) HIP_TRY(hipEventRecord(ix->mir_ev[0], s));

  PostingParams pp{};
  pp.offsets = bp.offsets;
  pp.live_map = bp.live_map;
  pp.n_docs = N;
  pp.C = C;
  pp.NC = S.NC;
  pp.crank = S.crank.as<uint2>();
  pp.range_shift = S.range_shift;
  pp.n_ranges = S.R;
  pp.n_blocks = S.n_blocks;
  pp.csr = bp.csr;
  pp.csr_esc = bp.csr_esc;
  pp.n_esc = S.h_esc.size();
  pp.rsplit = bp.rsplit;
  pp.doc_norm = bp.doc_norm;
  pp.blk = S.blk.as<uint32_t>();
  pp.bbase = S.bbase.as<uint64_t>();
  pp.post = S.post.as<uint32_t>();
  pp.post_tmp = ix->post_tmp.as<uint32_t>();
  pp.post_esc = S.post_esc.as<uint64_t>();
  pp.post_esc_count = reinterpret_cast<uint32_t *>(ctr + 10);
  pp.post_esc_cap = post_esc_cap;
  pp.sort_spw = sp.sort_spw;
  if (const char *e = knob("TFIDF_SORT_SPW")) pp.sort_spw = (uint32_t)std::max(1, std::min(8, atoi(e)));
  pp.err = bp.err;
  pp.first_block = first_block;
  pp.slices = sp.slices;
  pp.slice_docs = sp.slice_docs;
  pp.scan_parts = sp.scan_parts;
  pp.scan_width = sp.scan_width;
  pp.slice_cur = ix->inv_aux.as<uint32_t>();
  pp.part_tot = pp.slice_cur + (sp.slices > 1 ? (size_t)(S.n_blocks - first_block) * S.R * 64 : 0);
  pp.df_base = S.df_base.as<uint32_t>();
  pp.df_fold_end = dbp.fold_end;
  pp.df_from_rows = dbp.from_rows ? 1u : 0u;
  HIP_TRY(hipEventRecord(ix->ev[EV_D0], s));
  if (S.term_major) {
    TermParams tp{};
    if (N > kTermMaxDocs)
      return fail(TFIDF_E_CAPACITY, "the term-major layout holds at most 2^26 documents per shard");
    tp.offsets = bp.offsets;
    tp.live_map = bp.live_map;
    tp.n_docs = N;
    tp.nnz = S.nnz;
    tp.C = C;
    tp.slot_bits = ix->cap_log2;
    tp.doc_bits = 1;
    while ((1ull << tp.doc_bits) < N) tp.doc_bits++;
    tp.tf_bits = std::min(56u - tp.slot_bits - tp.doc_bits, 24u);
    if (const char *e = knob("TFIDF_TEST_TERM_TF_BITS"))
      tp.tf_bits = std::max(1u, std::min(tp.tf_bits, (uint32_t)atoi(e)));
    tp.csr = bp.csr;
    tp.csr_esc = bp.csr_esc;
    tp.n_esc = S.h_esc.size();
    tp.doc_nuniq = bp.doc_nuniq;
    tp.doc_norm = bp.doc_norm;
    tp.row_off = S.row_off.as<uint32_t>();
    HIP_TRY(ix->tvals.reserve_slack(S.nnz * 8 + 16));
    tp.keys = ix->post_tmp.as<uint64_t>();
    tp.keys_alt = ix->tvals.as<uint64_t>();
    tp.post = S.post.as<uint64_t>();
    tp.toff = S.toff.as<uint64_t>();
    tp.df = S.tdf.as<uint32_t>();
    tp.err = bp.err;
    tp.tesc_cap = row_cap / ((1u << tp.tf_bits) - 1) + 64;
    HIP_TRY(ix->term_esc.reserve(tp.tesc_cap * 16));
    tp.tesc = ix->term_esc.as<uint64_t>();
    tp.tesc_count = reinterpret_cast<uint32_t *>(ctr + 12);
    HIP_TRY(ix->term_tmp.reserve(term_invert_scratch_words(N, S.nnz, C) * 4));
    tp.scratch = ix->term_tmp.as<uint32_t>();
    HIP_TRY(hipEventRecord(ix->ev[EV_DF], s));
    HIP_TRY(hipEventRecord(ix->ev[EV_BSCAN], s));
    HIP_TRY(hipEventRecord(ix->ev[EV_CSCAN], s));
    HIP_TRY(launch_term_pairs(tp, s));
    {
      uint32_t ne = 0;
      HIP_TRY(hipMemcpyAsync(&ne, tp.tesc_count, 4, hipMemcpyDeviceToHost, s));
      HIP_TRY(commit_sync(ix, s));
      if (ne > tp.tesc_cap) return fail(TFIDF_E_CAPACITY, "term-major escape list overflow");
      if (ne) {
        std::vector<std::pair<uint64_t, uint64_t>> h(ne);
        ix->prof.stream_syncs++;
        HIP_TRY(hipMemcpy(h.data(), tp.tesc, ne * 16, hipMemcpyDeviceToHost));
        std::sort(h.begin(), h.end());
        HIP_TRY(hipMemcpy(tp.tesc, h.data(), ne * 16, hipMemcpyHostToDevice));
      }
      tp.n_tesc = ne;
    }
    HIP_TRY(launch_term_sort(tp, s));
    HIP_TRY(hipEventRecord(ix->ev[EV_SCAT], s));
  } else {
    if (inv.remap) HIP_TRY(launch_blk_remap(pp, blk_old, df_old, S.crank_inv.as<uint2>(), S.NC_inv, s));
    if (S.n_blocks) {
      HIP_TRY(launch_inv_zero(pp, s));
      HIP_TRY(launch_df_partial(pp, s));
    } else {
      HIP_TRY(hipMemsetAsync(S.blk.p, 0, (size_t)S.NC * 4, s));
    }
    HIP_TRY(hipEventRecord(ix->ev[EV_DF], s));
    HIP_TRY(launch_df_sum(pp, s));
    if (dict_delta || df_delta) {
      MirrorDeltaParams dp{};
      dp.crank = S.crank.as<uint2>();
      dp.crank_inv = S.crank_inv.as<uint2>();
      dp.df_col = S.blk.as<uint32_t>() + (size_t)S.n_blocks * S.NC;
      dp.C = C;
      dp.df_slot = S.sdf.as<uint32_t>();
      dp.dict = S.dict.as<uint64_t>();
      dp.dict_list = dict_delta ? ix->mir_dict_list.as<DictDelta>() : nullptr;
      dp.dict_cap = mp.n_new;
      dp.dict_count = reinterpret_cast<uint32_t *>(ctr + 15);
      dp.df_list = df_delta ? ix->mir_df_list.as<DfDelta>() : nullptr;
      dp.df_cap = df_cap;
      dp.df_count = reinterpret_cast<uint32_t *>(ctr + 14);
      HIP_TRY(launch_df_slots_delta(dp, s));
    } else if (!keep_sdf) {
      HIP_TRY(launch_df_slots(S.crank.as<uint2>(), S.blk.as<uint32_t>() + (size_t)S.n_blocks * S.NC, C,
                              S.sdf.as<uint32_t>(), s));
    }
    if (side_work) HIP_TRY(hipEventRecord(ix->mir_ev[2], s));
    if (S.n_blocks) HIP_TRY(launch_row_scan(pp, s));
    HIP_TRY(hipEventRecord(ix->ev[EV_BSCAN], s));
    HIP_TRY(launch_block_base(pp, s));
    HIP_TRY(hipEventRecord(ix->ev[EV_CSCAN], s));
    if (S.n_blocks) HIP_TRY(launch_scatter(pp, s));
    HIP_TRY(hipEventRecord(ix->ev[EV_SCAT], s));
  }
  if (side_work) {
    HIP_TRY(hipStreamWaitEvent(ix->copy_stream, ix->mir_ev[0], 0));
    if (dict_whole)
      HIP_TRY(hipMemcpyAsync(S.h_dict.data(), S.dict.p, (size_t)2 * C * 8, hipMemcpyDeviceToHost, ix->copy_stream));
    HIP_TRY(launch_verify_deferred(bp, ix->copy_stream));
    if (S.term_major)
      HIP_TRY(launch_count_nonzero(S.dict.as<uint64_t>(), C, reinterpret_cast<unsigned long long *>(ctr + 7),
                                   ix->copy_stream));
    if (!S.term_major) {
      HIP_TRY(hipStreamWaitEvent(ix->copy_stream, ix->mir_ev[2], 0));
      if (df_whole)
        HIP_TRY(hipMemcpyAsync(S.h_df.data(), S.df_dev(), (size_t)C * 4, hipMemcpyDeviceToHost, ix->copy_stream));
      HIP_TRY(S.h_crank.resize((size_t)C / 32 + 1));
      if (crank_whole)
        HIP_TRY(hipMemcpyAsync(S.h_crank.data(), S.crank.p, ((size_t)C / 32 + 1) * 8, hipMemcpyDeviceToHost,
                               ix->copy_stream));
      if (dict_delta)
        HIP_TRY(hipMemcpyAsync(ix->h_dict_delta.data(), ix->mir_dict_list.p, (size_t)mp.n_new * sizeof(DictDelta),
                               hipMemcpyDeviceToHost, ix->copy_stream));
    }
    HIP_TRY(hipEventRecord(ix->mir_ev[1], ix->copy_stream));
  }
  {
    tfidf_host_profile &pf = ix->prof;
    pf.mirror_dict = mp.dict;
    pf.mirror_df = mp.df;
    pf.mirror_crank = S.term_major ? (uint32_t)TFIDF_MIRROR_NONE : (uint32_t)mp.crank;
    if (dict_whole) pf.bytes_dict += (uint64_t)2 * C * 8;
    if (dict_delta) pf.bytes_dict += (uint64_t)mp.n_new * sizeof(DictDelta);
    if (df_whole) pf.bytes_df += (uint64_t)C * 4;
    if (crank_whole && !S.term_major) pf.bytes_crank += ((uint64_t)C / 32 + 1) * 8;
    pf.dict_delta_entries = dict_delta ? mp.n_new : 0;
    pf.df_delta_entries = 0;
  }
  if (!mirror_side && dict_whole)
    HIP_TRY(hipMemcpyAsync(S.h_dict.data(), S.dict.p, (size_t)2 * C * 8, hipMemcpyDeviceToHost, s));
  if ((!mirror_side || S.term_major) && df_whole)
    HIP_TRY(hipMemcpyAsync(S.h_df.data(), S.df_dev(), (size_t)C * 4, hipMemcpyDeviceToHost, s));
  if (!S.term_major && !mirror_side) {
    HIP_TRY(S.h_crank.resize((size_t)C / 32 + 1));
    if (crank_whole)
      HIP_TRY(hipMemcpyAsync(S.h_crank.data(), S.crank.p, ((size_t)C / 32 + 1) * 8, hipMemcpyDeviceToHost, s));
    if (dict_delta)
      HIP_TRY(hipMemcpyAsync(ix->h_dict_delta.data(), ix->mir_dict_list.p, (size_t)mp.n_new * sizeof(DictDelta),
                             hipMemcpyDeviceToHost, s));
  }
  if (side_work) {
    HIP_TRY(hipStreamWaitEvent(s, ix->mir_ev[1], 0));
  } else if (!mirror_side) {
    HIP_TRY(launch_verify_deferred(bp, s));
    if (S.term_major)
      HIP_TRY(launch_count_nonzero(S.dict.as<uint64_t>(), C, reinterpret_cast<unsigned long long *>(ctr + 7), s));
  }
  uint64_t tail[13];
  HIP_TRY(hipMemcpyAsync(tail, ctr + 3, sizeof tail, hipMemcpyDeviceToHost, s));
  if (!S.term_major) {
    HIP_TRY(S.h_bbase.resize((size_t)S.n_blocks + 2));
    HIP_TRY(hipMemcpyAsync(S.h_bbase.data(), S.bbase.p, ((size_t)S.n_blocks + 1) * 8, hipMemcpyDeviceToHost, s));
  }
  ix->prof.ms_enqueued = prof_ms(ix);
  HIP_TRY(commit_sync(ix, s));
  ix->prof.ms_synced = prof_ms(ix);
  {
    const EscAppend pe = esc_append_bounds(kept_pe, S.term_major ? 0 : (uint32_t)tail[7], post_esc_cap);
    if (pe.overflow) return fail(TFIDF_E_CAPACITY, "posting escape list overflow");
    const uint64_t n_pe = pe.first + pe.count;
    S.h_post_esc.resize(n_pe);
    if (pe.count) {
      ix->prof.stream_syncs++;
      HIP_TRY(hipMemcpy(S.h_post_esc.data() + pe.first, S.post_esc.as<uint64_t>() + pe.first, pe.count * 8,
                        hipMemcpyDeviceToHost));
      esc_merge(&S.h_post_esc, pe.first);
      HIP_TRY(hipMemcpy(S.post_esc.p, S.h_post_esc.data(), n_pe * 8, hipMemcpyHostToDevice));
    }
  }
  if (const uint32_t n_bad = (uint32_t)tail[5]) {
    std::vector<uint32_t> bad(n_bad);
    ix->prof.stream_syncs++;
    HIP_TRY(hipMemcpy(bad.data(), ix->bad_list.p, (size_t)n_bad * 4, hipMemcpyDeviceToHost));
    merge_malformed(&S.malformed, bad.data(), n_bad);
  }
  const uint32_t err2 = (uint32_t)tail[0];
  if (err2 & kErrCollision) { ix->collision_doc = (uint32_t)(tail[0] >> 32); return kRcCollision; }
  if (err2 & kErrTfTooLarge) return fail(TFIDF_E_UNSUPPORTED_INPUT, "a term frequency exceeds 2^24 - 1");
  if (dict_delta) {
    if ((uint32_t)tail[12] != mp.n_new)
      return fail(TFIDF_E_STATE, "dictionary mirror delta: %u new slots listed, %u expected", (uint32_t)tail[12],
                  mp.n_new);
    if (!apply_dict_delta(S.h_dict.data(), C, ix->h_dict_delta.data(), mp.n_new))
      return fail(TFIDF_E_STATE, "dictionary mirror delta names a slot past the dictionary");
  }
  if (df_delta) {
    const uint32_t n_df = (uint32_t)tail[11];
    if (n_df > df_cap) {
      ix->prof.stream_syncs++;
      HIP_TRY(hipMemcpy(S.h_df.data(), S.df_dev(), (size_t)C * 4, hipMemcpyDeviceToHost));
      ix->prof.mirror_df = TFIDF_MIRROR_WHOLE;
      ix->prof.bytes_df += (uint64_t)C * 4;
    } else {
      if (n_df) {
        HIP_TRY(hipMemcpyAsync(ix->h_df_delta.data(), ix->mir_df_list.p, (size_t)n_df * sizeof(DfDelta),
                               hipMemcpyDeviceToHost, s));
        HIP_TRY(commit_sync(ix, s));
        if (!apply_df_delta(S.h_df.data(), C, ix->h_df_delta.data(), n_df))
          return fail(TFIDF_E_STATE, "df mirror delta names a slot past the dictionary");
      }
      ix->prof.bytes_df += (uint64_t)n_df * sizeof(DfDelta);
      ix->prof.df_delta_entries = n_df;
    }
  }
  S.num_terms = keep_rank ? S.NC : tail[4];

  tfidf_commit_timing &t = ix->timing;
  t.ms_tokenize = ev_ms(ix, EV_START, EV_TOK);
  t.ms_long = n_long ? ev_ms(ix, EV_L0, EV_LONG) : 0.0f;
  t.ms_df = ev_ms(ix, EV_D0, EV_DF);
  t.ms_blockscan = ev_ms(ix, EV_DF, EV_BSCAN);
  t.ms_colscan = ev_ms(ix, EV_BSCAN, EV_CSCAN);
  t.ms_scatter = ev_ms(ix, EV_CSCAN, EV_SCAT);
  t.ms_total = t.ms_tokenize + t.ms_long + ev_ms(ix, EV_D0, EV_SCAT);
  t.text_bytes = ix->text_bytes;
  t.num_docs = N;
  t.nnz = S.nnz;

  S.cap_log2 = ix->cap_log2;
  S.text_bytes = ix->text_bytes;
  S.text = ix->text;
  S.offsets = ix->offsets;
  ix->keys.compact();
  S.keys = ix->keys;
  S.hash_seed = ix->hash_seed;
  S.sig = sig;
  {
    std::lock_guard<std::mutex> tl(S.term_mu);
    S.term_cache.clear();
  }
  {
    std::lock_guard<std::mutex> ml(S.mlt_mu);
    S.mlt_ready = false;
  }
  S.mir_ok = true;
  S.tok_docs = ix->n_staged;
  if (!S.term_major) {
    S.inv_docs = ix->n_staged;
    S.NC_inv = S.NC;
// ... 9 lines not shown
  ix->prof_t0 = std::chrono::steady_clock::now();
  struct Wall {
    tfidf_index *ix;
    ~Wall() { ix->prof.ms_wall = prof_ms(ix); }
  } wall{ix};
  if (ix->compact_pct && ix->n_dead && ix->dead_bytes * 100 >= (uint64_t)ix->compact_pct * ix->text_bytes)
    compact_locked(ix, nullptr, nullptr);
  std::shared_ptr<Snapshot> S;
  if (ix->spare && ix->spare.use_count() == 1) S = std::move(ix->spare);
  ix->spare.reset();
  if (!S) S = std::make_shared<Snapshot>(ix->cfg.device);
  const char *weak = knob("TFIDF_TEST_WEAK_HASH");
  ix->hash_seed = ix->hash_floor ? ix->hash_floor : ((weak && atoi(weak)) ? kWeakHashSeed : 0);
  ix->hash_rebuilds = ix->hash_floor;
  for (uint32_t attempt = ix->hash_floor;; attempt++) {
    int rc = commit_once(ix, *S, attempt == ix->hash_floor);
    if (rc != TFIDF_OK) {
      hipStreamSynchronize(ix->stream);
      hipStreamSynchronize(ix->copy_stream);
    }
    if (rc == kRcCollision) {
      if (attempt == 3) {
        ix->spare = std::move(S);
        return fail(TFIDF_E_UNSUPPORTED_INPUT, "hash collisions under 4 seeds (last in document %u)", ix->collision_doc);
      }
      ix->hash_seed = attempt + 1;
      ix->hash_rebuilds++;
      continue;
    }
    if (rc != TFIDF_OK) {
      ix->spare = std::move(S);
      return rc == kRcNoPublish ? TFIDF_OK : rc;
    }
    S->hash_rebuilds = ix->hash_rebuilds;
    S->generation = ++ix->generation;
    {
      std::lock_guard<std::mutex> sl(ix->snap_mu);
      std::swap(ix->cur, S);
    }
    ix->prof.ms_published = prof_ms(ix);
    ix->spare = std::move(S);
    return TFIDF_OK;
  }
}

extern "C" int tfidf_set_hash_attempt(tfidf_index *ix, uint32_t attempt) {
  if (!ix) return fail(TFIDF_E_INVALID_ARG, "NULL index");
  if (attempt > 3) return fail(TFIDF_E_INVALID_ARG, "hash seed attempt %u > 3", attempt);
  std::lock_guard<std::mutex> lk(ix->mu);
  ix->hash_floor = attempt;
  return TFIDF_OK;
}

extern "C" int tfidf_commit_tokenized_docs(const tfidf_index *ix, uint64_t *docs, uint32_t *was_full) {
  if (!ix) return fail(TFIDF_E_INVALID_ARG, "NULL index");
  std::lock_guard<std::mutex> lk(const_cast<tfidf_index *>(ix)->mu);
  if (docs) *docs = ix->last_tok_docs;
  if (was_full) *was_full = ix->last_tok_full;
  return TFIDF_OK;
}

extern "C" int tfidf_commit_host_profile(const tfidf_index *ix, tfidf_host_profile *out) {
  if (!ix || !out) return fail(TFIDF_E_INVALID_ARG, "NULL argument");
  std::lock_guard<std::mutex> lk(const_cast<tfidf_index *>(ix)->mu);
  *out = ix->prof;
  return TFIDF_OK;
}

extern "C" int tfidf_commit_inverted_blocks(const tfidf_index *ix, uint32_t *first_block, uint32_t *n_blocks,
                                            uint32_t *remapped) {
  if (!ix) return fail(TFIDF_E_INVALID_ARG, "NULL index");
  std::lock_guard<std::mutex> lk(const_cast<tfidf_index *>(ix)->mu);
  if (first_block) *first_block = ix->last_inv_first;
  if (n_blocks) *n_blocks = ix->last_inv_blocks;
  if (remapped) *remapped = ix->last_inv_remap;
  return TFIDF_OK;
}

extern "C" int tfidf_commit_inversion_shape(const tfidf_index *ix, uint32_t *slices, uint32_t *scan_parts) {
  if (!ix) return fail(TFIDF_E_INVALID_ARG, "NULL index");
  std::lock_guard<std::mutex> lk(const_cast<tfidf_index *>(ix)->mu);
  if (slices) *slices = ix->last_inv_slices;
  if (scan_parts) *scan_parts = ix->last_inv_scan_parts;
  return TFIDF_OK;
}

extern "C" int tfidf_get_commit_timing(const tfidf_index *ix, tfidf_commit_timing *out) {
  if (!ix || !out) return fail(TFIDF_E_INVALID_ARG, "NULL argument");
  *out = ix->timing;
  return TFIDF_OK;
}

extern "C" int tfidf_stats(const tfidf_index *ix, tfidf_index_stats *out) {
  if (!ix || !out) return fail(TFIDF_E_INVALID_ARG, "NULL argument");
  const std::shared_ptr<Snapshot> S = current(ix);
  *out = tfidf_index_stats{};
  uint64_t staged_bytes = 0;
  {
    std::lock_guard<std::mutex> lk(const_cast<tfidf_index *>(ix)->mu);
    out->text_bytes = ix->text_bytes;
    out->hash_seed = ix->hash_seed;
    out->hash_rebuilds = ix->hash_rebuilds;
    staged_bytes = ix->text->bytes + ix->offsets->bytes;
    out->dead_docs = ix->n_dead;
    out->dead_bytes = ix->dead_bytes;
    out->compactions = ix->compactions;
  }
  if (S) {
    out->num_docs = S->n_docs;
    out->doc_count = S->doc_count;
    out->sum_ttf = S->sum_ttf;
    out->num_terms = S->num_terms;
    out->nnz = S->nnz;
    out->long_docs = S->long_docs;
    out->term_major = S->term_major;
    out->pack_docs = S->pack_docs;
    out->pack_retried = S->pack_retried;
    out->unicode_docs = S->unicode_docs;
    out->unicode_wave_docs = S->unicode_wave_docs;
    out->long_chunked = S->long_chunked;
    out->malformed_docs = S->malformed.size();
    out->hash_seed = S->hash_seed;
    out->hash_rebuilds = S->hash_rebuilds;
  }
  {
    std::lock_guard<std::mutex> cl(ix->cq_mu);
    out->coalesced_batches = ix->cq_batches;
    out->coalesced_queries = ix->cq_queries;
  }
  out->unit_batches = ix->unit_batches.load();
  out->fused_queries = ix->fused_queries.load();
  out->unit_count = ix->unit_count.load();
  uint64_t tot = staged_bytes;
  if (S) {
    const DevBuf *bufs[] = {&S->dict, &S->csr, &S->csr_esc, &S->doc_len, &S->doc_nuniq, &S->doc_norm,
                            &S->rsplit, &S->blk, &S->bbase, &S->post, &S->toff, &S->tdf, &S->crank, &S->sdf,
                            &S->crank_inv, &S->blk_alt, &S->df_base, &S->df_base_alt};
    for (const DevBuf *b : bufs) tot += b->bytes;
  }
  out->device_bytes = tot;
  return TFIDF_OK;
}


static uint32_t host_lookup(const Snapshot &S, uint64_t lo, uint64_t hi) {
  if (S.C == 0) return kInvalidSlot;
  const uint32_t mask = S.C - 1;
  uint32_t s = dict_home(dict_hash(lo, hi), mask) & ~1u;
  for (uint32_t it = 0; it <= mask; it++) {
    const uint64_t clo = S.h_dict[s], chi = S.h_dict[(size_t)S.C + s];
    if (clo == 0) return kInvalidSlot;
    if (clo == lo && chi == hi) return s;
    s = (s + 1) & mask;
  }
  return kInvalidSlot;
}

struct StrSink {
  std::string s;
  void push(uint8_t c) { s.push_back((char)c); }
};
static int slot_term(Snapshot &S, uint32_t slot, std::string *out) {
  char b[32];
  const uint64_t lo = S.h_dict[slot], hi = S.h_dict[(size_t)S.C + slot];
  if (const uint32_t n = key_decode(lo, hi, b)) { out->assign(b, n); return TFIDF_OK; }
  std::lock_guard<std::mutex> tl(S.term_mu);
// ... 4242 lines not shown
```

tf-idf-distributed-system_amd/csrc/tfidf_internal.h:

```cpp
#pragma once

#include <hip/hip_runtime.h>
#include <stdint.h>
#include <stdlib.h>

#include <atomic>
#include <string>
#include <vector>

#include "tfidf_common.h"

namespace tfidf {

inline const char *knob(const char *name) {
  const char *d = getenv("TFIDF_DEBUG");
  if (!d || !*d || (d[0] == '0' && !d[1])) return nullptr;
  return getenv(name);
}

constexpr uint32_t kErrCapacity = 4u;
constexpr uint32_t kErrTfTooLarge = 8u;
constexpr uint32_t kErrLongScratch = 16u;
constexpr uint32_t kErrCollision = 32u;

// ... 82 lines not shown
#include "unicode_scan.h"
#endif
namespace tfidf {
#if defined(__HIPCC__)
typedef const BuildParams __attribute__((address_space(4))) KBuildParams;
__device__ __forceinline__ KBuildParams *cold_args() {
  KBuildParams *q = (KBuildParams *)__builtin_amdgcn_kernarg_segment_ptr();
  asm volatile("" : "+s"(q));
  return q;
}
#define TFIDF_COLD(f) (cold_args()->f)

__device__ inline void set_build_err(uint32_t *err, uint32_t flag, uint32_t doc) {
  const uint32_t old = atomicOr(err, flag);
  if (old == 0) atomicExch(err + 1, doc);
}
__device__ inline void dict_verify(const BuildParams &p, uint32_t slot, uint64_t mine, uint32_t doc) {
  const uint64_t r = __hip_atomic_load(p.dict + 2 * ((size_t)p.cap_mask + 1) + slot, __ATOMIC_RELAXED,
                                       __HIP_MEMORY_SCOPE_AGENT);
  if (r == mine) return;
  if (r == 0) {
    const uint32_t at = atomicAdd(TFIDF_COLD(verify_count), 1u);
    if (at < TFIDF_COLD(verify_cap)) {
      uint64_t *vd = TFIDF_COLD(verify_defer);
      vd[2 * (size_t)at] = slot;
      vd[2 * (size_t)at + 1] = mine;
    } else {
      set_build_err(TFIDF_COLD(err), kErrCollision, doc);
    }
    return;
  }
  if (!uc_same_term(p.text + dict_ref_off(r), dict_ref_len(r), p.text + dict_ref_off(mine), dict_ref_len(mine)))
    set_build_err(TFIDF_COLD(err), kErrCollision, doc);
}

__device__ inline void csr_put(const BuildParams &p, uint64_t idx, uint32_t slot, uint32_t tf, uint32_t doc) {
  const uint32_t esc = csr_esc_value(p.range_shift);
  uint32_t f = tf;
  if (tf >= esc) {
    f = esc;
    if (tf > kMaxTf) set_build_err(TFIDF_COLD(err), kErrTfTooLarge, doc);
    const uint32_t at = atomicAdd(TFIDF_COLD(esc_count), 1u);
    if (at < TFIDF_COLD(esc_cap)) TFIDF_COLD(csr_esc)[at] = (idx << 24) | (tf > kMaxTf ? kMaxTf : tf);
  }
  __builtin_nontemporal_store(csr_local(slot, p.range_shift) | (f << p.range_shift), p.csr + idx);
}
#endif

constexpr uint32_t kPostTfEsc = 2047;
__host__ __device__ inline uint32_t post_word(uint32_t doc_local, uint32_t tf, uint32_t norm) {
  return doc_local | ((tf < kPostTfEsc ? tf : kPostTfEsc) << 13) | (norm << 24);
}

struct PostingParams {
  const uint64_t *offsets;
  const uint32_t *live_map;
  uint64_t n_docs;
  uint32_t C;
  uint32_t range_shift, n_ranges;
  uint32_t n_blocks;
  const uint32_t *csr, *rsplit;
  const uint64_t *csr_esc;
  uint64_t n_esc;
  const uint8_t *doc_norm;
  uint32_t NC;
  const uint2 *crank;
  uint32_t *blk;
  uint64_t *bbase;
  uint32_t *post;
  uint64_t *post_esc;
  uint32_t *post_esc_count;
  uint64_t post_esc_cap;
  uint32_t *err;
  uint32_t *post_tmp;
  uint32_t sort_spw;
  uint32_t first_block;
  uint32_t slices, slice_docs;
  uint32_t scan_parts, scan_width;
  uint32_t *slice_cur;
  uint32_t *part_tot;
  uint32_t *df_base;
  uint32_t df_fold_end;
  uint32_t df_from_rows;
};

inline void allow_dyn_lds(const void *fn, int bytes, std::atomic<uint64_t> &done_mask) {
  int dev = 0;
  hipGetDevice(&dev);
  const uint64_t bit = 1ull << (dev & 63);
  if (done_mask.load(std::memory_order_acquire) & bit) return;
  hipFuncSetAttribute(fn, hipFuncAttributeMaxDynamicSharedMemorySize, bytes);
  done_mask.fetch_or(bit, std::memory_order_acq_rel);
}

hipError_t launch_tokenize_wave(const BuildParams &p, int grid, hipStream_t s);
hipError_t launch_doc_range(uint32_t *list, uint32_t *count, uint32_t first, uint32_t n, hipStream_t s);
hipError_t launch_tokenize_wave_uni(const BuildParams &p, int grid, hipStream_t s);
hipError_t launch_tokenize_chunks_uni(const BuildParams &p, int grid, hipStream_t s);
constexpr uint32_t kWaveWGsPerCU = 8;
constexpr uint32_t kWaveGroups = 128;
constexpr uint32_t kPackMaxDocs = 16;
constexpr uint64_t kPackBytes = 2560;
hipError_t launch_tokenize_long(const BuildParams &p, int grid, hipStream_t s);
constexpr uint32_t kLongCoreBytes = 2048;
constexpr uint64_t kPairBudget = 2ull << 30;
constexpr uint32_t kPairWords = 512;
#ifndef TFIDF_LR_WIN_BITS
#define TFIDF_LR_WIN_BITS 15
#define TFIDF_LR_THREADS 1024
#endif
#ifndef TFIDF_LR_IN
#define TFIDF_LR_IN 16
#define TFIDF_LR_UPT 2
#endif
#ifdef TFIDF_LR_WPE
#define TFIDF_LR_ATTR __attribute__((amdgpu_waves_per_eu(TFIDF_LR_WPE)))
#else
#define TFIDF_LR_ATTR
#endif
constexpr uint32_t kLrWinBits = TFIDF_LR_WIN_BITS;
constexpr uint32_t kLrWin = 1u << kLrWinBits;
constexpr uint32_t kLrThreads = TFIDF_LR_THREADS;
static_assert(kLrWinBits <= kRangeBits && kLrWin / kLrThreads <= 32 && kLrWin / kLrThreads >= 4, "k_long_rows window");
constexpr uint32_t kPairTfBits = 12;
hipError_t launch_tokenize_chunks(const BuildParams &p, int grid, hipStream_t s);
hipError_t launch_long_rows(const BuildParams &p, uint32_t n_docs, hipStream_t s);
hipError_t launch_tokenize_uwave(const BuildParams &p, int grid, hipStream_t s);
hipError_t launch_tokenize_uchunk(const BuildParams &p, int grid, hipStream_t s);
constexpr uint32_t kUwaveWGsPerCU = 7;
constexpr uint32_t kUchunkWGsPerCU = 8;
hipError_t launch_verify_deferred(const BuildParams &p, hipStream_t s);
hipError_t launch_inv_zero(const PostingParams &p, hipStream_t s);
hipError_t launch_df_partial(const PostingParams &p, hipStream_t s);
hipError_t launch_df_sum(const PostingParams &p, hipStream_t s);
hipError_t launch_row_scan(const PostingParams &p, hipStream_t s);
hipError_t launch_block_base(const PostingParams &p, hipStream_t s);
hipError_t launch_count_nonzero(const uint64_t *a, uint32_t n, unsigned long long *out, hipStream_t s);
hipError_t launch_col_rank(const uint64_t *dict_lo, uint32_t C, uint2 *crank, unsigned long long *n_cols, hipStream_t s);
hipError_t launch_df_slots(const uint2 *crank, const uint32_t *df_col, uint32_t C, uint32_t *df_slot, hipStream_t s);
struct DictDelta;
struct DfDelta;
struct MirrorDeltaParams {
  const uint2 *crank, *crank_inv;
  const uint32_t *df_col;
  uint32_t C;
  uint32_t *df_slot;
  const uint64_t *dict;
  DictDelta *dict_list;
  uint32_t dict_cap;
  uint32_t *dict_count;
  DfDelta *df_list;
  uint32_t df_cap;
  uint32_t *df_count;
};
hipError_t launch_df_slots_delta(const MirrorDeltaParams &p, hipStream_t s);
hipError_t launch_scatter(const PostingParams &p, hipStream_t s);
hipError_t launch_blk_remap(const PostingParams &p, const uint32_t *blk_old, const uint32_t *df_old,
                            const uint2 *crank_inv, uint32_t NC_inv, hipStream_t s);

constexpr uint64_t kTermMaxDocs = 1ull << 26;
struct TermParams {
  const uint64_t *offsets;
  const uint32_t *live_map;
  uint64_t n_docs, nnz;
  uint32_t C, slot_bits;
  uint32_t doc_bits, tf_bits;
  const uint32_t *csr, *doc_nuniq;
  const uint64_t *csr_esc;
  uint64_t n_esc;
  const uint8_t *doc_norm;
  uint32_t *row_off;
  uint64_t *keys, *keys_alt;
  uint64_t *tesc;
  uint32_t *tesc_count;
  uint64_t tesc_cap, n_tesc;
  uint32_t *scratch;
  uint64_t *post;
  uint64_t *toff;
  uint32_t *df;
  uint32_t *err;
};
uint64_t term_invert_scratch_words(uint64_t n_docs, uint64_t nnz, uint32_t C);
hipError_t launch_term_pairs(const TermParams &p, hipStream_t s);
hipError_t launch_term_sort(const TermParams &p, hipStream_t s);

constexpr uint32_t kInlTerms = 32;
constexpr uint32_t kFusedMaxK = 64;
struct QueryParams {
  const uint64_t *post;
  const uint32_t *post32;
  const uint64_t *post_esc;
  uint64_t n_post_esc;
  const uint64_t *bbase;
  const uint32_t *blk;
  const uint64_t *toff;
  uint32_t C;
  uint32_t n_blocks;
  uint64_t n_docs;
  const float *cache;
  const uint32_t *q_off;
  const uint32_t *q_slot;
  const float *q_w;
  const uint32_t *q_role;
  const uint32_t *q_meta;
  uint32_t ops;
  uint32_t n_q;
  uint32_t q_chunk;
  uint32_t k;
  uint64_t *cand;
  uint32_t *cand_n;
  uint32_t *out_doc;
  float *out_score;
  uint32_t *out_n;
  uint64_t *hits;
  uint32_t *hits_n;
  uint32_t hits_R2;
  uint32_t *ovf_list;
// ... 305 lines not shown
```

tf-idf-distributed-system_amd/tfidf_amd/_lib.py:

```python
import ctypes as C
import os
import subprocess

PKG_ROOT = os.path.dirname(os.path.dirname(os.path.abspath(__file__)))
LIB_PATH = os.path.join(PKG_ROOT, "lib", "libtfidf.so")

OK = 0
E_INVALID_ARG = 1
E_HIP = 2
E_OOM = 3
E_UNSUPPORTED_INPUT = 4
E_UNSUPPORTED_QUERY = 5
E_CAPACITY = 6
E_STATE = 7
E_BUFFER = 8
E_NO_DEVICE = 9
E_QUERY_SYNTAX = 10

STATS_SHARD = 0
STATS_GLOBAL = 1

OWN_STREAM = C.c_void_p(-1 & ((1 << 64) - 1))

INVERSION_AUTO = 0
# ... 129 lines not shown
                                U64P, F32P]),
    "tfidf_reader_snippets": (C.c_int, [VP, C.c_char_p, C.c_uint64, U32P, C.c_uint64, C.c_uint32, VP, C.c_uint64,
                                        U64P, U64P, U64P, U32P, U32P, C.c_uint64, U64P, U64P, U64P, F32P]),
    "tfidf_snippets": (C.c_int, [VP, C.c_char_p, C.c_uint64, U32P, C.c_uint64, C.c_uint32, VP, C.c_uint64, U64P,
                                 U64P, U64P, U32P, U32P, C.c_uint64, U64P, U64P, U64P, F32P]),
    "tfidf_reader_matches_batch": (C.c_int, [VP, C.c_char_p, U64P, C.c_uint32, U32P, U64P, U64P, U32P, U32P,
                                             C.c_uint64, U64P, U64P, F32P]),
    "tfidf_matches_batch": (C.c_int, [VP, C.c_char_p, U64P, C.c_uint32, U32P, U64P, U64P, U32P, U32P, C.c_uint64,
                                      U64P, U64P, F32P]),
    "tfidf_reader_snippets_batch": (C.c_int, [VP, C.c_char_p, U64P, C.c_uint32, U32P, U64P, C.c_uint32, VP,
                                              C.c_uint64, U64P, U64P, U64P, U32P, U32P, C.c_uint64, U64P, U64P,
                                              U64P, F32P]),
    "tfidf_snippets_batch": (C.c_int, [VP, C.c_char_p, U64P, C.c_uint32, U32P, U64P, C.c_uint32, VP, C.c_uint64,
                                       U64P, U64P, U64P, U32P, U32P, C.c_uint64, U64P, U64P, U64P, F32P]),
    "tfidf_last_highlight_chunks": (C.c_int, [VP, U64P, U64P]),
    "tfidf_fuzzy_terms_batch": _fuzzy_batch_sig(U32P),
    "tfidf_reader_fuzzy_terms_batch": _fuzzy_batch_sig(U32P),
    "tfidf_fuzzy_terms": _FUZZY_SINGLE_SIG,
    "tfidf_reader_fuzzy_terms": _FUZZY_SINGLE_SIG,
    "tfidf_last_fuzzy_chunks": (C.c_int, [VP, U64P, U64P]),
    "tfidf_fuzzy_expand_batch": _FUZZY_EXPAND_BATCH_SIG,
    "tfidf_reader_fuzzy_expand_batch": _FUZZY_EXPAND_BATCH_SIG,
    "tfidf_fuzzy_expand": _FUZZY_EXPAND_SINGLE_SIG,
    "tfidf_reader_fuzzy_expand": _FUZZY_EXPAND_SINGLE_SIG,
    "tfidf_search_fuzzy_batch": _fuzzy_search_batch_sig(U32P),
    "tfidf_reader_search_fuzzy_batch": _fuzzy_search_batch_sig(U32P),
    "tfidf_node_search_fuzzy_batch": _fuzzy_search_batch_sig(U64P),
    "tfidf_search_fuzzy": _FUZZY_SEARCH_SINGLE_SIG,
    "tfidf_reader_search_fuzzy": _FUZZY_SEARCH_SINGLE_SIG,
    "tfidf_wildcard_terms_batch": _wildcard_terms_sig(U32P),
    "tfidf_reader_wildcard_terms_batch": _wildcard_terms_sig(U32P),
    "tfidf_node_wildcard_terms_batch": _wildcard_terms_sig(U64P),
    "tfidf_wildcard_terms": _WILDCARD_TERMS_SINGLE_SIG,
    "tfidf_reader_wildcard_terms": _WILDCARD_TERMS_SINGLE_SIG,
    "tfidf_search_wildcard_batch": _wildcard_docs_sig(U32P),
    "tfidf_reader_search_wildcard_batch": _wildcard_docs_sig(U32P),
    "tfidf_node_search_wildcard_batch": _wildcard_docs_sig(U64P),
    "tfidf_search_wildcard": _WILDCARD_DOCS_SINGLE_SIG,
    "tfidf_reader_search_wildcard": _WILDCARD_DOCS_SINGLE_SIG,
    "tfidf_last_wildcard_stats": (C.c_int, [VP, U64P, U64P, U64P]),
    "tfidf_regex_terms_batch": _wildcard_terms_sig(U32P),
    "tfidf_reader_regex_terms_batch": _wildcard_terms_sig(U32P),
    "tfidf_node_regex_terms_batch": _wildcard_terms_sig(U64P),
    "tfidf_regex_terms": _WILDCARD_TERMS_SINGLE_SIG,
    "tfidf_reader_regex_terms": _WILDCARD_TERMS_SINGLE_SIG,
    "tfidf_search_regex_batch": _wildcard_docs_sig(U32P),
    "tfidf_reader_search_regex_batch": _wildcard_docs_sig(U32P),
    "tfidf_node_search_regex_batch": _wildcard_docs_sig(U64P),
    "tfidf_search_regex": _WILDCARD_DOCS_SINGLE_SIG,
    "tfidf_reader_search_regex": _WILDCARD_DOCS_SINGLE_SIG,
    "tfidf_last_regex_stats": (C.c_int, [VP, U64P, U64P, U64P, U64P]),
    "tfidf_search_phrase_batch": (C.c_int, [VP, C.c_char_p, U64P, C.c_uint32, U32P, F32P, U32P, C.c_uint64, U64P,
                                            U64P]),
    "tfidf_reader_search_phrase_batch": (C.c_int, [VP, C.c_char_p, U64P, C.c_uint32, U32P, F32P, U32P, C.c_uint64,
                                                   U64P, U64P]),
    "tfidf_search_phrase": (C.c_int, [VP, C.c_char_p, C.c_uint64, U32P, F32P, U32P, C.c_uint64, U64P]),
    "tfidf_reader_search_phrase": (C.c_int, [VP, C.c_char_p, C.c_uint64, U32P, F32P, U32P, C.c_uint64, U64P]),
    "tfidf_node_search_phrase_batch": (C.c_int, [VP, C.c_char_p, U64P, C.c_uint32, U64P, F32P, U32P, C.c_uint64,
                                                 U64P, U64P]),
    "tfidf_last_phrase_stats": (C.c_int, [VP, U64P, U64P]),
    "tfidf_search_phrase_slop_batch": (C.c_int, [VP, C.c_char_p, U64P, U32P, C.c_uint32, U32P, F32P, F32P, C.c_uint64,
                                                 U64P, U64P]),
    "tfidf_reader_search_phrase_slop_batch": (C.c_int, [VP, C.c_char_p, U64P, U32P, C.c_uint32, U32P, F32P, F32P,
                                                        C.c_uint64, U64P, U64P]),
    "tfidf_search_phrase_slop": (C.c_int, [VP, C.c_char_p, C.c_uint64, C.c_uint32, U32P, F32P, F32P, C.c_uint64, U64P]),
    "tfidf_reader_search_phrase_slop": (C.c_int, [VP, C.c_char_p, C.c_uint64, C.c_uint32, U32P, F32P, F32P, C.c_uint64,
                                                  U64P]),
    "tfidf_node_search_phrase_slop_batch": (C.c_int, [VP, C.c_char_p, U64P, U32P, C.c_uint32, U64P, F32P, F32P,
                                                      C.c_uint64, U64P, U64P]),
    "tfidf_mlt_params_init": (C.c_int, [MLTP]),
    "tfidf_mlt_terms_batch": _MLT_TERMS_SIG,
    "tfidf_reader_mlt_terms_batch": _MLT_TERMS_SIG,
    "tfidf_more_like_this_batch": _MLT_BATCH_SIG,
    "tfidf_reader_more_like_this_batch": _MLT_BATCH_SIG,
    "tfidf_more_like_this": _MLT_SINGLE_SIG,
    "tfidf_reader_more_like_this": _MLT_SINGLE_SIG,
    "tfidf_last_mlt_stats": (C.c_int, [VP, U64P, U64P]),
    "tfidf_query_positive_terms": (C.c_int, [C.c_char_p, C.c_uint64, C.c_char_p, C.c_uint64, U64P, U64P]),
    "tfidf_set_hash_attempt": (C.c_int, [VP, C.c_uint32]),
    "tfidf_get_commit_timing": (C.c_int, [VP, C.POINTER(CommitTiming)]),
    "tfidf_commit_tokenized_docs": (C.c_int, [VP, U64P, U32P]),
    "tfidf_commit_inverted_blocks": (C.c_int, [VP, U32P, U32P, U32P]),
    "tfidf_commit_inversion_shape": (C.c_int, [VP, U32P, U32P]),
    "tfidf_commit_host_profile": (C.c_int, [VP, C.POINTER(HostProfile)]),
    "tfidf_stats": (C.c_int, [VP, C.POINTER(IndexStats)]),
    "tfidf_search": (C.c_int, [VP, C.c_char_p, C.c_uint64, C.c_uint32, U32P, F32P, C.c_uint64, U64P]),
    "tfidf_search_coalesced": (C.c_int, [VP, C.c_char_p, C.c_uint64, C.c_uint32, U32P, F32P, C.c_uint64, U64P,
                                         C.c_uint32]),
    "tfidf_search_batch": (C.c_int, [VP, C.c_char_p, U64P, C.c_uint32, C.c_uint32, U32P, F32P, U32P]),
    "tfidf_search_batch_all": (C.c_int, [VP, C.c_char_p, U64P, C.c_uint32, U32P, F32P, C.c_uint64, U64P, U64P]),
    "tfidf_reader_search_batch_all": (C.c_int, [VP, C.c_char_p, U64P, C.c_uint32, U32P, F32P, C.c_uint64, U64P,
                                                U64P]),
    "tfidf_last_search_ms": (C.c_int, [VP, F32P, F32P]),
    "tfidf_set_query_timing": (C.c_int, [VP, C.c_int]),
    "tfidf_search_batch_keys_device": (C.c_int, [VP, C.c_char_p, U64P, C.c_uint32, C.c_uint32, C.c_uint64, VP]),
    "tfidf_search_all_keys_device": (C.c_int, [VP, C.c_char_p, C.c_uint64, C.c_uint64, VP, C.c_uint64, U64P]),
    "tfidf_set_stream": (C.c_int, [VP, VP]),
    "tfidf_doc_keys": (C.c_int, [VP, C.c_char_p, C.c_uint64, U64P, U64P]),
    "tfidf_sort_names": (C.c_int, [C.c_char_p, U64P, C.c_uint64, U64P]),
    "tfidf_doc_key": (C.c_int, [VP, C.c_uint64, C.c_char_p, C.c_uint64, U64P]),
    "tfidf_doc_len": (C.c_int, [VP, C.c_uint64, U32P, U8P]),
    "tfidf_malformed_docs": (C.c_int, [VP, U64P, C.c_uint64, U64P]),
    "tfidf_doc_terms": (C.c_int, [VP, C.c_uint64, C.c_char_p, C.c_uint64, U32P, C.c_uint64, U64P]),
    "tfidf_term_df": (C.c_int, [VP, C.c_char_p, C.c_uint64, U64P, U64P]),
    "tfidf_vocab_size": (C.c_int, [VP, U64P]),
    "tfidf_vocab_export": (C.c_int, [VP, U64P, U32P, U32P, C.c_uint64, U64P]),
    "tfidf_vocab_export_device": (C.c_int, [VP, VP, VP, C.c_uint64, U64P]),
    "tfidf_vocab_canonicalize_device": (C.c_int, [VP, VP, C.c_uint64, VP, C.c_uint64, U64P]),
    "tfidf_set_global_stats_device": (C.c_int, [VP, VP, C.c_uint64, C.c_uint64, C.c_uint64]),
    "tfidf_vocab_partition_device": (C.c_int, [VP, C.c_uint32, VP, C.c_uint64, VP, U64P]),
    "tfidf_vocab_reduce_device": (C.c_int, [VP, VP, C.c_uint64, VP, VP]),
    "tfidf_set_global_df_device": (C.c_int, [VP, VP, C.c_uint64, C.c_uint64, C.c_uint64]),
    "tfidf_set_global_stats": (C.c_int, [VP, U64P, U64P, C.c_uint64, C.c_uint64, C.c_uint64]),
    "tfidf_clear_global_stats": (C.c_int, [VP]),
    "tfidf_term_key": (C.c_int, [C.c_char_p, C.c_uint64, U64P, U64P]),
    "tfidf_analyze": (C.c_int, [C.c_char_p, C.c_uint64, C.c_char_p, C.c_uint64, U64P, U64P]),
    "tfidf_leader_merge": (C.c_int, [C.c_char_p, U64P, C.c_uint64, F64P, U64P, F64P, U64P]),
    "tfidf_synth_corpus": (C.c_int, [C.c_int, C.c_uint64, C.c_uint64, C.c_uint64, F64P, C.c_uint32, C.c_uint32,
                                     C.c_uint32, C.POINTER(VP), C.POINTER(VP), U64P]),
    "tfidf_comm_create": (C.c_int, [C.c_int32, C.c_int32, VP, C.POINTER(VP)]),
    "tfidf_rccl_unique_id": (C.c_int, [VP]),
    "tfidf_comm_init_rccl": (C.c_int, [VP, C.c_int32, C.c_int32, C.c_int32, C.POINTER(VP)]),
    "tfidf_comm_create_inproc": (C.c_int, [C.c_int32, C.POINTER(VP)]),
    "tfidf_comm_destroy": (C.c_int, [VP]),
    "tfidf_comm_info": (C.c_int, [VP, C.POINTER(C.c_int32), C.POINTER(C.c_int32), C.POINTER(C.c_int32)]),
    "tfidf_comm_selftest": (C.c_int, [VP]),
    "tfidf_dist_global_commit": (C.c_int, [VP, VP, U64P, U64P, U64P]),
    "tfidf_dist_search": (C.c_int, [VP, VP, C.c_uint64, C.c_char_p, C.c_uint64, C.c_uint32, U64P, F32P, C.c_uint64,
                                    U64P]),
    "tfidf_dist_search_batch": (C.c_int, [VP, VP, C.c_uint64, C.c_char_p, U64P, C.c_uint32, C.c_uint32, U64P, F32P,
                                          U32P]),
    "tfidf_dist_shard_commit": (C.c_int, [VP, VP, U64P]),
    "tfidf_dist_shard_search": (C.c_int, [VP, VP, C.c_char_p, C.c_uint64, U64P, U64P]),
    "tfidf_dist_search_batch_all": (C.c_int, [VP, VP, C.c_uint64, C.c_char_p, U64P, C.c_uint32, U64P, F32P, C.c_uint64,
                                              U64P, U64P]),
    "tfidf_dist_shard_search_batch": (C.c_int, [VP, VP, C.c_char_p, U64P, C.c_uint32, U64P, U64P]),
    "tfidf_dist_last_names_batch": (C.c_int, [VP, C.c_char_p, C.c_uint64, U64P, F64P, C.c_uint64, U64P, U64P, U64P]),
    "tfidf_dist_last_hits": (C.c_int, [VP, U64P, F32P, C.c_uint64, U64P]),
    "tfidf_dist_last_failed": (C.c_int, [VP, U64P]),
    "tfidf_reader_open": (C.c_int, [VP, C.POINTER(VP)]),
    "tfidf_reader_close": (C.c_int, [VP]),
    "tfidf_reader_info": (C.c_int, [VP, U64P, U64P]),
    "tfidf_reader_search": (C.c_int, [VP, C.c_char_p, C.c_uint64, C.c_uint32, U32P, F32P, C.c_uint64, U64P]),
    "tfidf_reader_doc_key": (C.c_int, [VP, C.c_uint64, C.c_char_p, C.c_uint64, U64P]),
    "tfidf_reader_doc_keys": (C.c_int, [VP, C.c_char_p, C.c_uint64, U64P, U64P]),
    "tfidf_dist_last_names": (C.c_int, [VP, C.c_char_p, C.c_uint64, U64P, F64P, C.c_uint64, U64P, U64P]),
    "tfidf_node_create": (C.c_int, [VP, C.c_uint64, C.POINTER(VP)]),
    "tfidf_node_create_devices": (C.c_int, [VP, C.POINTER(C.c_int32), C.c_uint32, C.c_uint32, C.POINTER(VP)]),
    "tfidf_node_destroy": (C.c_int, [VP]),
    "tfidf_node_shard": (C.c_int, [VP, C.c_uint32, C.POINTER(VP), U32P]),
    "tfidf_node_add_docs": (C.c_int, [VP, C.c_int32, C.c_char_p, U64P, C.c_uint64, C.c_char_p, U64P]),
    "tfidf_node_commit": (C.c_int, [VP]),
    "tfidf_node_delete_docs": (C.c_int, [VP, C.c_int32, C.c_char_p, U64P, C.c_uint64, U64P]),
    "tfidf_node_compact": (C.c_int, [VP, U64P]),
    "tfidf_node_search": (C.c_int, [VP, C.c_char_p, C.c_uint64, C.c_uint32, U64P, F32P, C.c_uint64, U64P]),
    "tfidf_node_search_batch": (C.c_int, [VP, C.c_char_p, U64P, C.c_uint32, C.c_uint32, U64P, F32P, U32P]),
    "tfidf_node_search_names": (C.c_int, [VP, C.c_char_p, C.c_uint64, C.c_char_p, C.c_uint64, U64P, F64P,
                                          C.c_uint64, U64P, U64P]),
    "tfidf_node_search_batch_all": (C.c_int, [VP, C.c_char_p, U64P, C.c_uint32, U64P, F32P, C.c_uint64, U64P, U64P]),
    "tfidf_node_search_names_batch": (C.c_int, [VP, C.c_char_p, U64P, C.c_uint32, U64P, U64P]),
    "tfidf_node_last_names_batch": (C.c_int, [VP, C.c_char_p, C.c_uint64, U64P, F64P, C.c_uint64, U64P, U64P, U64P]),
    "tfidf_node_doc_key": (C.c_int, [VP, C.c_uint64, C.c_char_p, C.c_uint64, U64P]),
    "tfidf_node_matches_batch": (C.c_int, [VP, C.c_char_p, U64P, C.c_uint32, U64P, U64P, U64P, U32P, U32P,
                                           C.c_uint64, U64P, U64P, F32P]),
    "tfidf_node_snippets_batch": (C.c_int, [VP, C.c_char_p, U64P, C.c_uint32, U64P, U64P, C.c_uint32, VP, C.c_uint64,
                                            U64P, U64P, U64P, U32P, U32P, C.c_uint64, U64P, U64P, U64P, F32P]),
# ... 46 lines not shown
```

tf-idf-distributed-system_amd/tfidf_amd/engine.py:

```python
import ctypes as C
import os

import numpy as np

from . import _lib as L


def analyze(text: bytes):
    cap = 2 * len(text) + 64
    buf = C.create_string_buffer(cap)
    nt, nb = C.c_uint64(), C.c_uint64()
    L.check(L.load().tfidf_analyze(text, len(text), buf, cap, C.byref(nt), C.byref(nb)))
    return buf.raw[:nb.value].split(b"\0")[:nt.value]


def term_key(term: bytes):
    lo, hi = C.c_uint64(), C.c_uint64()
    L.check(L.load().tfidf_term_key(term, len(term), C.byref(lo), C.byref(hi)))
    return lo.value, hi.value


def _batch_all_arrays(fn, handle, queries, cap):
    nq = len(queries)
    offs = np.zeros(nq + 1, np.uint64)
# ... 711 lines not shown
        a, b, c, d = C.c_uint64(), C.c_uint64(), C.c_uint64(), C.c_uint64()
        L.check(L.load().tfidf_last_regex_stats(self._h, C.byref(a), C.byref(b), C.byref(c), C.byref(d)))
        return a.value, b.value, c.value, d.value

    def last_fuzzy_chunks(self):
        a, b = C.c_uint64(), C.c_uint64()
        L.check(L.load().tfidf_last_fuzzy_chunks(self._h, C.byref(a), C.byref(b)))
        return a.value, b.value

    def search_phrase(self, phrase: bytes):
        return _phrase_single(L.load().tfidf_search_phrase, self._h, phrase)

    def search_phrase_batch_arrays(self, phrases, cap=None):
        return _phrase_batch_arrays(L.load().tfidf_search_phrase_batch, self._h, phrases, cap)

    def search_phrase_batch(self, phrases):
        return _phrase_lists(*self.search_phrase_batch_arrays(phrases))

    def search_phrase_slop(self, phrase: bytes, slop: int):
        return _phrase_single(L.load().tfidf_search_phrase_slop, self._h, phrase, int(slop))

    def search_phrase_slop_batch_arrays(self, phrases, slops, cap=None):
        return _phrase_batch_arrays(L.load().tfidf_search_phrase_slop_batch, self._h, phrases, cap, slops=slops)

    def search_phrase_slop_batch(self, phrases, slops):
        return _phrase_lists(*self.search_phrase_slop_batch_arrays(phrases, slops))

    def last_phrase_stats(self):
        a, b = C.c_uint64(), C.c_uint64()
        L.check(L.load().tfidf_last_phrase_stats(self._h, C.byref(a), C.byref(b)))
        return a.value, b.value

    def more_like_this(self, doc, k=10, exclude_seed=True, **params):
        return _mlt_single(L.load().tfidf_more_like_this, self._h, doc, k, exclude_seed, mlt_params(**params))

    def more_like_this_batch_arrays(self, docs, k=10, exclude_seed=True, **params):
        return _mlt_batch_arrays(L.load().tfidf_more_like_this_batch, self._h, docs, k, exclude_seed,
                                 mlt_params(**params))

    def more_like_this_batch(self, docs, k=10, exclude_seed=True, **params):
        return _topk_lists(*self.more_like_this_batch_arrays(docs, k, exclude_seed, **params))

    def mlt_terms_batch_arrays(self, docs, term_cap=None, bytes_cap=None, **params):
        return _mlt_terms_arrays(L.load().tfidf_mlt_terms_batch, self._h, docs, mlt_params(**params), term_cap,
                                 bytes_cap)

    def mlt_terms_batch(self, docs, **params):
        return _mlt_terms_lists(self.mlt_terms_batch_arrays(docs, **params))

    def mlt_terms_arrays(self, doc, **params):
        return self.mlt_terms_batch_arrays([doc], **params)

    def mlt_terms(self, doc, **params):
        return self.mlt_terms_batch([doc], **params)[0]

    def last_mlt_stats(self):
        a, b = C.c_uint64(), C.c_uint64()
        L.check(L.load().tfidf_last_mlt_stats(self._h, C.byref(a), C.byref(b)))
        return a.value, b.value

    def set_hash_attempt(self, attempt):
        L.check(L.load().tfidf_set_hash_attempt(self._h, attempt))

    def commit_timing(self):
        t = L.CommitTiming()
        L.check(L.load().tfidf_get_commit_timing(self._h, C.byref(t)))
        return {f: getattr(t, f) for f, _ in L.CommitTiming._fields_}

    def commit_tokenized_docs(self):
        n, full = C.c_uint64(), C.c_uint32()
        L.check(L.load().tfidf_commit_tokenized_docs(self._h, C.byref(n), C.byref(full)))
        return {"docs": n.value, "was_full": bool(full.value)}

    def commit_inverted_blocks(self):
        f, n, r = C.c_uint32(), C.c_uint32(), C.c_uint32()
        L.check(L.load().tfidf_commit_inverted_blocks(self._h, C.byref(f), C.byref(n), C.byref(r)))
        return {"first_block": f.value, "n_blocks": n.value, "remapped": r.value}

    def commit_inversion_shape(self):
        s, p = C.c_uint32(), C.c_uint32()
        L.check(L.load().tfidf_commit_inversion_shape(self._h, C.byref(s), C.byref(p)))
        return {"slices": s.value, "scan_parts": p.value}

    def commit_host_profile(self):
        p = L.HostProfile()
        L.check(L.load().tfidf_commit_host_profile(self._h, C.byref(p)))
        out = {f: getattr(p, f) for f, _ in L.HostProfile._fields_}
        for m in ("mirror_dict", "mirror_df", "mirror_crank"):
            out[m] = L.MIRROR_FORMS[out[m]]
        return out

    def stats(self):
        s = L.IndexStats()
        L.check(L.load().tfidf_stats(self._h, C.byref(s)))
        return {f: getattr(s, f) for f, _ in L.IndexStats._fields_}

    def search(self, query: bytes, k=0):
        if k == 0:
            with self.reader() as rd:
                return rd.search(query, 0)
        lib = L.load()
        docs = np.zeros(k, np.uint32)
        scores = np.zeros(k, np.float32)
        n = C.c_uint64()
        rc = lib.tfidf_search(self._h, query, len(query), k, L.ptr(docs, C.c_uint32), L.ptr(scores, C.c_float),
                              k, C.byref(n))
        L.check(rc)
        m = n.value
        return list(zip(docs[:m].tolist(), scores[:m].tolist()))

    def reader(self):
        return Reader(self)

    def search_coalesced(self, query: bytes, k, wait_us=50, cap=None):
        if cap is None:
            cap = k if k else max(self.stats()["num_docs"], 1)
        docs = np.empty(max(cap, 1), np.uint32)
        scores = np.empty(max(cap, 1), np.float32)
        n = C.c_uint64()
        L.check(L.load().tfidf_search_coalesced(self._h, query, len(query), k, L.ptr(docs, C.c_uint32),
                                                L.ptr(scores, C.c_float), cap, C.byref(n), wait_us))
        m = n.value
        return list(zip(docs[:m].tolist(), scores[:m].tolist()))

    def search_batch_all_arrays(self, queries, cap=None):
        if cap is None:
            cap = min(65536 * max(len(queries), 1), 1 << 24)
        return _batch_all_arrays(L.load().tfidf_search_batch_all, self._h, queries, cap)

    def search_batch_all(self, queries):
        return _hit_lists(*self.search_batch_all_arrays(queries))

    def search_all_arrays(self, query: bytes):
        with self.reader() as rd:
            return rd.search_arrays(query, 0)

    def search_arrays(self, query: bytes, k):
        lib = L.load()
        docs = np.zeros(max(k, 1), np.uint32)
        scores = np.zeros(max(k, 1), np.float32)
        n = C.c_uint64()
        L.check(lib.tfidf_search(self._h, query, len(query), k, L.ptr(docs, C.c_uint32), L.ptr(scores, C.c_float),
                                 max(k, 1), C.byref(n)))
        return docs[:n.value], scores[:n.value]

    def search_batch(self, queries, k):
        nq = len(queries)
        offs = np.zeros(nq + 1, np.uint64)
        offs[1:] = np.cumsum([len(q) for q in queries], dtype=np.uint64)
        docs = np.zeros((nq, k), np.uint32)
        scores = np.zeros((nq, k), np.float32)
        counts = np.zeros(nq, np.uint32)
        L.check(L.load().tfidf_search_batch(self._h, b"".join(queries), L.ptr(offs, C.c_uint64), nq, k,
                                            L.ptr(docs, C.c_uint32), L.ptr(scores, C.c_float),
                                            L.ptr(counts, C.c_uint32)))
        return docs, scores, counts

    def search_batch_keys_device(self, queries, k, doc_base, d_keys):
        nq = len(queries)
        offs = np.zeros(nq + 1, np.uint64)
        offs[1:] = np.cumsum([len(q) for q in queries], dtype=np.uint64)
        L.check(L.load().tfidf_search_batch_keys_device(self._h, b"".join(queries), L.ptr(offs, C.c_uint64), nq, k,
                                                        doc_base, C.c_void_p(d_keys)))

    def search_all_keys_device(self, query: bytes, doc_base, d_keys, cap):
        n = C.c_uint64()
# ... 338 lines not shown
```

Before: 7.959 billion.

## Fuse df count, df sum, row scan and block base into one last-block-done kernel

Adds k_df_fused, which counts per-range df in LDS, accumulates counts into a global scratch, and lets the last-arriving workgroup per range (ticket counter) do the prefix scan, the df fold and the block base. It replaces the separate inv_zero, df_partial, df_sum, row_scan and block_base launches when exactly one new block is inverted with several slices. The aim is to cut kernel launches and intermediate per-slice round trips. In exchange it adds agent-scope atomics and fences, a scratch buffer that must be kept zeroed, and a serial scan done by a single workgroup per range.

```diff
diff --git a/include/tfidf.h b/include/tfidf.h
--- a/include/tfidf.h
+++ b/include/tfidf.h
@@ -112,6 +112,7 @@
 int tfidf_commit_inverted_blocks(const tfidf_index *ix, uint32_t *first_block, uint32_t *n_blocks,
                                  uint32_t *remapped);
 int tfidf_commit_inversion_shape(const tfidf_index *ix, uint32_t *slices, uint32_t *scan_parts);
+int tfidf_commit_inversion_fused(const tfidf_index *ix, uint32_t *fused);
 int tfidf_commit_host_profile(const tfidf_index *ix, tfidf_host_profile *out);
 
 int tfidf_delete_docs(tfidf_index *ix, const uint8_t *keys, const uint64_t *key_offsets, uint64_t n_keys,
diff --git a/tf-idf-distributed-system_amd/csrc/commit_plan.h b/tf-idf-distributed-system_amd/csrc/commit_plan.h
--- a/tf-idf-distributed-system_amd/csrc/commit_plan.h
+++ b/tf-idf-distributed-system_amd/csrc/commit_plan.h
@@ -212,6 +212,54 @@
 }
 
 
+inline bool fuse_plan(bool term_major, uint32_t inv_blocks, const SlicePlan &sp, const char *rows_knob,
+                      const char *parts_knob, const char *unfused_knob) {
+  auto on = [](const char *v) { return v && *v && !(v[0] == '0' && !v[1]); };
+  if (term_major || inv_blocks != 1 || sp.slices < 2) return false;
+  if (on(rows_knob) || on(unfused_knob)) return false;
+  if (parts_knob && *parts_knob) return false;
+  return true;
+}
+
+inline uint32_t fuse_tickets(const SlicePlan &sp, uint64_t docs) {
+  if (docs == 0 || sp.slice_docs == 0) return 0;
+  return (uint32_t)std::min<uint64_t>(sp.slices, (docs + sp.slice_docs - 1) / sp.slice_docs);
+}
+
+TFIDF_PLAN_HD uint32_t fuse_ctl_words(uint32_t R) { return (2 * R + 1 + 63) / 64 * 64; }
+inline uint64_t fuse_scratch_words(uint32_t R, uint32_t NC) { return (uint64_t)fuse_ctl_words(R) + NC; }
+
+struct FuseScratch {
+  uint64_t words = 0;
+  bool clean = false;
+};
+inline bool fuse_scratch_must_zero(const FuseScratch &s, uint64_t need, bool *grow) {
+  *grow = need > s.words;
+  return *grow || !s.clean;
+}
+inline void fuse_scratch_launch(FuseScratch *s, uint64_t words) { s->words = words; s->clean = false; }
+inline void fuse_scratch_done(FuseScratch *s) { s->clean = true; }
+
+inline uint64_t fuse_range_start(const uint32_t *rsplit, uint64_t n_docs, uint32_t R, uint32_t r) {
+  uint64_t s = 0;
+  if (r)
+    for (uint64_t d = 0; d < n_docs; d++) s += rsplit[d * R + r - 1];
+  return s;
+}
+inline uint64_t fuse_block_total(const uint32_t *rsplit, uint64_t n_docs, uint32_t R) {
+  uint64_t s = 0;
+  for (uint64_t d = 0; d < n_docs; d++) s += rsplit[d * R + R - 1];
+  return s;
+}
+inline uint64_t fuse_range_offsets(const uint32_t *counts, uint32_t c0, uint32_t c1, uint64_t start, uint32_t *offsets) {
+  for (uint32_t c = c0; c < c1; c++) {
+    offsets[c] = (uint32_t)start;
+    start += counts[c];
+  }
+  return start;
+}
+
+
 enum MirrorForm : uint32_t { kMirrorNone = 0, kMirrorDelta = 1, kMirrorWhole = 2 };
 
 constexpr uint32_t kDictDeltaDiv = 32;
diff --git a/tf-idf-distributed-system_amd/csrc/kernels_index.hip b/tf-idf-distributed-system_amd/csrc/kernels_index.hip
--- a/tf-idf-distributed-system_amd/csrc/kernels_index.hip
+++ b/tf-idf-distributed-system_amd/csrc/kernels_index.hip
@@ -2114,16 +2114,21 @@
 };
 
 template <int Q>
-__device__ __forceinline__ InvQuads<Q> inv_quads(const PostingParams &p, uint64_t dd, uint64_t d1, uint32_t r) {
+__device__ __forceinline__ InvQuads<Q> inv_quads_lohi(const PostingParams &p, uint64_t dd, uint64_t d1, uint32_t r,
+                                                      uint32_t *lo_out, uint32_t *hi_out) {
   const uint32_t lane = threadIdx.x & 63;
   const uint64_t d = dd + lane;
   uint64_t at = 0;
   uint32_t n = 0;
+  *lo_out = *hi_out = 0;
   if (lane < (uint32_t)(4 * Q) && d < d1) {
     const uint64_t src = p.live_map ? p.live_map[d] : d;
     const uint32_t lo = r ? p.rsplit[d * p.n_ranges + r - 1] : 0;
+    const uint32_t hi = p.rsplit[d * p.n_ranges + r];
     at = csr_row_base(p.offsets, src) + lo;
-    n = p.rsplit[d * p.n_ranges + r] - lo;
+    n = hi - lo;
+    *lo_out = lo;
+    *hi_out = hi;
   }
   InvQuads<Q> g;
 #pragma unroll
@@ -2134,6 +2139,11 @@
     g.n[q] = (uint32_t)__shfl((int)n, from, 64);
   }
   return g;
+}
+template <int Q>
+__device__ __forceinline__ InvQuads<Q> inv_quads(const PostingParams &p, uint64_t dd, uint64_t d1, uint32_t r) {
+  uint32_t lo, hi;
+  return inv_quads_lohi<Q>(p, dd, d1, r, &lo, &hi);
 }
 
 template <int Q>
@@ -2167,6 +2177,47 @@
 }
 static uint32_t tiles_grid(uint32_t n_blocks, uint32_t R) { return (n_blocks + 7) / 8 * 8 * R; }
 
+template <bool SUMS>
+__device__ __forceinline__ void df_count_docs(const PostingParams &p, uint32_t *hist, uint64_t d0, uint64_t d1, uint32_t r,
+                                              uint32_t *lo_sum, uint32_t *hi_sum) {
+  const uint32_t nw = blockDim.x >> 6;
+  const uint32_t wid = (uint32_t)__builtin_amdgcn_readfirstlane((int)(threadIdx.x >> 6));
+  const uint32_t rmask = (1u << p.range_shift) - 1;
+  constexpr int Q = kDfQuads, E = 4 * Q;
+  const uint64_t step = (uint64_t)nw * E;
+  uint64_t dd = d0 + (uint64_t)wid * E;
+  uint32_t lo, hi, los, his;
+  InvQuads<Q> cur = inv_quads_lohi<Q>(p, dd, d1, r, &los, &his);
+  uint32_t c[E];
+  inv_load<Q>(p, cur, 0, c);
+  auto count = [&](uint32_t e) __attribute__((always_inline)) {
+    const uint32_t sl = e & rmask;
+    atomicAdd(&hist[sl >> 1], 1u << ((sl & 1u) << 4));
+  };
+  while (dd < d1) {
+    const uint64_t dn = dd + step;
+    const InvQuads<Q> nxt = inv_quads_lohi<Q>(p, dn, d1, r, &lo, &hi);
+    if (SUMS) { los += lo; his += hi; }
+    uint32_t cn[E];
+    inv_load<Q>(p, nxt, 0, cn);
+#pragma unroll
+    for (int j = 0; j < E; j++)
+      if (c[j]) count(c[j]);
+    const uint32_t maxn = inv_maxn<Q>(cur);
+    for (uint32_t off = 64; __any(off < maxn); off += 64) {
+      inv_load<Q>(p, cur, off, c);
+#pragma unroll
+      for (int j = 0; j < E; j++)
+        if (c[j]) count(c[j]);
+    }
+    cur = nxt;
+#pragma unroll
+    for (int j = 0; j < E; j++) c[j] = cn[j];
+    dd = dn;
+  }
+  if (SUMS) { *lo_sum = los; *hi_sum = his; }
+}
+
 template <bool SLICED>
 __global__ void __launch_bounds__(1024) k_df_partial(PostingParams p) {
   extern __shared__ uint32_t hist[];
@@ -2187,39 +2238,7 @@
   }
   for (uint32_t i = threadIdx.x; i < RS / 2; i += blockDim.x) hist[i] = 0;
   __syncthreads();
-  const uint32_t nw = blockDim.x >> 6;
-  const uint32_t wid = (uint32_t)__builtin_amdgcn_readfirstlane((int)(threadIdx.x >> 6));
-  const uint32_t rmask = RS - 1;
-  constexpr int Q = kDfQuads, E = 4 * Q;
-  const uint64_t step = (uint64_t)nw * E;
-  uint64_t dd = d0 + (uint64_t)wid * E;
-  InvQuads<Q> cur = inv_quads<Q>(p, dd, d1, r);
-  uint32_t c[E];
-  inv_load<Q>(p, cur, 0, c);
-  auto count = [&](uint32_t e) __attribute__((always_inline)) {
-    const uint32_t sl = e & rmask;
-    atomicAdd(&hist[sl >> 1], 1u << ((sl & 1u) << 4));
-  };
-  while (dd < d1) {
-    const uint64_t dn = dd + step;
-    const InvQuads<Q> nxt = inv_quads<Q>(p, dn, d1, r);
-    uint32_t cn[E];
-    inv_load<Q>(p, nxt, 0, cn);
-#pragma unroll
-    for (int j = 0; j < E; j++)
-      if (c[j]) count(c[j]);
-    const uint32_t maxn = inv_maxn<Q>(cur);
-    for (uint32_t off = 64; __any(off < maxn); off += 64) {
-      inv_load<Q>(p, cur, off, c);
-#pragma unroll
-      for (int j = 0; j < E; j++)
-        if (c[j]) count(c[j]);
-    }
-    cur = nxt;
-#pragma unroll
-    for (int j = 0; j < E; j++) c[j] = cn[j];
-    dd = dn;
-  }
+  df_count_docs<false>(p, hist, d0, d1, r, nullptr, nullptr);
   __syncthreads();
   uint32_t *out = p.blk + (size_t)b * p.NC;
   const uint32_t w0 = (r << p.range_shift) >> 5;
@@ -2661,6 +2680,152 @@
   if (tid == 0 && p.first_block == 0) p.bbase[0] = 0;
 }
 
+__global__ void __launch_bounds__(1024) k_df_fused(PostingParams p) {
+  extern __shared__ uint32_t hist[];
+  __shared__ uint32_t wsum[16];
+  __shared__ uint32_t carry_sh, sums_sh[2], last_sh;
+  uint32_t slice, r;
+  if (!tile_of(blockIdx.x, p.slices, p.n_ranges, &slice, &r)) return;
+  const uint32_t b = p.first_block;
+  const uint32_t R = p.n_ranges, RS = 1u << p.range_shift;
+  const uint32_t tid = threadIdx.x, lane = tid & 63, wid = tid >> 6;
+  uint64_t d0 = (uint64_t)b * kBlockDocs;
+  uint64_t d1 = d0 + kBlockDocs < p.n_docs ? d0 + kBlockDocs : p.n_docs;
+  d0 += (uint64_t)slice * p.slice_docs;
+  if (d0 >= d1) return;
+  d1 = d0 + p.slice_docs < d1 ? d0 + p.slice_docs : d1;
+  const uint32_t w0 = (r << p.range_shift) >> 5;
+  const uint32_t c0 = min(p.crank[w0].y, p.NC);
+  const uint32_t c1 = r + 1 < R ? min(p.crank[((r + 1) << p.range_shift) >> 5].y, p.NC) : p.NC;
+  for (uint32_t i = tid; i < RS / 2; i += blockDim.x) hist[i] = 0;
+  if (tid < 2) sums_sh[tid] = 0;
+  __syncthreads();
+  uint32_t lo_sum, hi_sum;
+  df_count_docs<true>(p, hist, d0, d1, r, &lo_sum, &hi_sum);
+  lo_sum = wave_sum(lo_sum);
+  hi_sum = wave_sum(hi_sum);
+  if (lane == 0) {
+    if (lo_sum) atomicAdd(&sums_sh[0], lo_sum);
+    if (hi_sum) atomicAdd(&sums_sh[1], hi_sum);
+  }
+  __syncthreads();
+  uint32_t *ctl = p.fuse, *cnt = p.fuse + fuse_ctl_words(R);
+  for (uint32_t w = tid; w < (RS >> 5); w += blockDim.x) {
+    const uint2 e = p.crank[w0 + w];
+    uint32_t bits = e.x, col = e.y;
+    while (bits) {
+      const uint32_t sl = 32 * w + (uint32_t)__builtin_ctz(bits);
+      bits &= bits - 1;
+      const uint32_t n = (hist[sl >> 1] >> ((sl & 1u) << 4)) & 0xFFFFu;
+      if (n) atomicAdd(&cnt[col], n);
+      col++;
+    }
+  }
+  if (tid == 0) {
+    if (sums_sh[0]) atomicAdd(&ctl[R + r], sums_sh[0]);
+    if (r + 1 == R && sums_sh[1]) atomicAdd(&ctl[2 * R], sums_sh[1]);
+  }
+  asm volatile("s_waitcnt vmcnt(0)" ::: "memory");
+  __syncthreads();
+  if (tid == 0) {
+    __builtin_amdgcn_fence(__ATOMIC_RELEASE, "agent");
+    asm volatile("s_waitcnt vmcnt(0)" ::: "memory");
+    const uint32_t t = __hip_atomic_fetch_add(&ctl[r], 1u, __ATOMIC_RELAXED, __HIP_MEMORY_SCOPE_AGENT);
+    last_sh = t + 1 == p.fuse_tickets ? 1u : 0u;
+  }
+  __syncthreads();
+  if (!last_sh) return;
+  if (tid == 0) {
+    __builtin_amdgcn_fence(__ATOMIC_ACQUIRE, "agent");
+    asm volatile("s_waitcnt vmcnt(0)" ::: "memory");
+  }
+  __syncthreads();
+  uint32_t start = 0;
+  if (tid == 0) start = __hip_atomic_load(&ctl[R + r], __ATOMIC_RELAXED, __HIP_MEMORY_SCOPE_AGENT);
+  const bool trusted = p.first_block != 0;
+  const bool fold = !p.first_block || p.df_fold_end > p.first_block;
+  const bool full_now = p.first_block < p.df_fold_end;
+  uint32_t *row = p.blk + (size_t)b * p.NC, *dfc = p.blk + (size_t)p.n_blocks * p.NC;
+  for (uint32_t t0 = c0; t0 < c1; t0 += 16384) {
+    const uint32_t i0 = t0 + tid * 16;
+    const bool whole = i0 + 16 <= c1;
+    uint32_t v[16], bs[16];
+    if (whole) {
+#pragma unroll
+      for (int q = 0; q < 4; q++) {
+        const csr_quad_t x = *reinterpret_cast<const csr_quad_t *>(cnt + i0 + 4 * q);
+        v[4 * q] = x.x; v[4 * q + 1] = x.y; v[4 * q + 2] = x.z; v[4 * q + 3] = x.w;
+      }
+#pragma unroll
+      for (int q = 0; q < 4; q++) {
+        csr_quad_t x = {0u, 0u, 0u, 0u};
+        if (trusted) x = *reinterpret_cast<const csr_quad_t *>(p.df_base + i0 + 4 * q);
+        bs[4 * q] = x.x; bs[4 * q + 1] = x.y; bs[4 * q + 2] = x.z; bs[4 * q + 3] = x.w;
+      }
+    } else {
+#pragma unroll
+      for (int q = 0; q < 16; q++) {
+        v[q] = i0 + q < c1 ? cnt[i0 + q] : 0u;
+        bs[q] = trusted && i0 + q < c1 ? p.df_base[i0 + q] : 0u;
+      }
+    }
+    uint32_t tot = 0;
+#pragma unroll
+    for (int q = 0; q < 16; q++) tot += v[q];
+    const uint32_t x = wave_incl_add(tot);
+    if (lane == 63) wsum[wid] = x;
+    if (tid == 0 && t0 == c0) carry_sh = start;
+    __syncthreads();
+    uint32_t base = carry_sh, all = 0;
+    for (uint32_t w = 0; w < 16; w++) {
+      const uint32_t sw = wsum[w];
+      if (w < wid) base += sw;
+      all += sw;
+    }
+    base += x - tot;
+    __syncthreads();
+    if (tid == 0) carry_sh += all;
+    uint32_t o[16];
+#pragma unroll
+    for (int q = 0; q < 16; q++) { o[q] = base; base += v[q]; }
+    if (whole) {
+      const csr_quad_t zero = {0u, 0u, 0u, 0u};
+#pragma unroll
+      for (int q = 0; q < 4; q++) {
+        const csr_quad_t vv = {v[4 * q], v[4 * q + 1], v[4 * q + 2], v[4 * q + 3]};
+        const csr_quad_t bb = {bs[4 * q], bs[4 * q + 1], bs[4 * q + 2], bs[4 * q + 3]};
+        const csr_quad_t oo = {o[4 * q], o[4 * q + 1], o[4 * q + 2], o[4 * q + 3]};
+        *reinterpret_cast<csr_quad_t *>(cnt + i0 + 4 * q) = zero;
+        *reinterpret_cast<csr_quad_t *>(dfc + i0 + 4 * q) = bb + vv;
+        if (fold) *reinterpret_cast<csr_quad_t *>(p.df_base + i0 + 4 * q) = full_now ? bb + vv : bb;
+        *reinterpret_cast<csr_quad_t *>(row + i0 + 4 * q) = oo;
+      }
+    } else {
+#pragma unroll
+      for (int q = 0; q < 16; q++)
+        if (i0 + q < c1) {
+          cnt[i0 + q] = 0;
+          dfc[i0 + q] = bs[q] + v[q];
+          if (fold) p.df_base[i0 + q] = full_now ? bs[q] + v[q] : bs[q];
+          row[i0 + q] = o[q];
+        }
+    }
+    __syncthreads();
+  }
+  if (tid < kPartStreams) p.slice_cur[(size_t)r * kPartStreams + tid] = 0;
+  if (tid == 0) {
+    __hip_atomic_store(&ctl[r], 0u, __ATOMIC_RELAXED, __HIP_MEMORY_SCOPE_AGENT);
+    __hip_atomic_store(&ctl[R + r], 0u, __ATOMIC_RELAXED, __HIP_MEMORY_SCOPE_AGENT);
+    if (r + 1 == R) {
+      const uint32_t total = __hip_atomic_load(&ctl[2 * R], __ATOMIC_RELAXED, __HIP_MEMORY_SCOPE_AGENT);
+      __hip_atomic_store(&ctl[2 * R], 0u, __ATOMIC_RELAXED, __HIP_MEMORY_SCOPE_AGENT);
+      const uint64_t bb = p.first_block ? p.bbase[b] : 0ull;
+      if (!p.first_block) p.bbase[0] = 0;
+      p.bbase[b + 1] = bb + total;
+    }
+  }
+}
+
 __global__ void __launch_bounds__(256) k_verify_deferred(BuildParams p) {
   const uint32_t n = min(*p.verify_count, p.verify_cap);
   const uint64_t *ref = p.dict + 2 * ((size_t)p.cap_mask + 1);
@@ -2774,6 +2939,16 @@
     hipLaunchKernelGGL(k_df_partial<true>, dim3(tiles_grid(nb * p.slices, p.n_ranges)), dim3(1024), lds, s, p);
   else
     hipLaunchKernelGGL(k_df_partial<false>, dim3(tiles_grid(nb, p.n_ranges)), dim3(1024), lds, s, p);
+  return hipGetLastError();
+}
+hipError_t launch_df_fused(const PostingParams &p, hipStream_t s) {
+  static std::atomic<uint64_t> done{0};
+  allow_dyn_lds((const void *)k_df_fused, 2 << kRangeBits, done);
+  if (p.n_blocks != p.first_block + 1 || p.slices < 2 || !p.fuse || !p.slice_cur || !p.df_base || p.df_from_rows ||
+      p.fuse_tickets == 0 || p.fuse_tickets > p.slices || p.df_fold_end < p.first_block || p.df_fold_end > p.n_blocks)
+    return hipErrorInvalidValue;
+  const size_t lds = (size_t)2 << p.range_shift;
+  hipLaunchKernelGGL(k_df_fused, dim3(tiles_grid(p.slices, p.n_ranges)), dim3(1024), lds, s, p);
   return hipGetLastError();
 }
 hipError_t launch_df_sum(const PostingParams &p, hipStream_t s) {
diff --git a/tf-idf-distributed-system_amd/csrc/tfidf_capi.hip b/tf-idf-distributed-system_amd/csrc/tfidf_capi.hip
--- a/tf-idf-distributed-system_amd/csrc/tfidf_capi.hip
+++ b/tf-idf-distributed-system_amd/csrc/tfidf_capi.hip
@@ -405,6 +405,7 @@
   uint32_t last_tok_full = 1;
   uint32_t last_inv_first = 0, last_inv_blocks = 0, last_inv_remap = 0;
   uint32_t last_inv_slices = 1, last_inv_scan_parts = 1;
+  uint32_t last_inv_fused = 0;
   tfidf_host_profile prof{};
   std::chrono::steady_clock::time_point prof_t0;
   uint64_t next_ord = 0;
@@ -418,6 +419,8 @@
   DevBuf new_list;
   DevBuf mir_dict_list, mir_df_list;
   DevBuf inv_aux;
+  DevBuf inv_fuse;
+  FuseScratch fuse_state;
   PinnedVec<DictDelta> h_dict_delta;
   PinnedVec<DfDelta> h_df_delta;
   DevBuf bad_list;
@@ -570,7 +573,7 @@
   ix->text.reset();
   ix->offsets.reset();
   DevBuf *bufs[] = {&ix->d_live_map, &ix->long_list, &ix->uni_list, &ix->counters, &ix->retry_list, &ix->new_list, &ix->bad_list,
-                    &ix->mir_dict_list, &ix->mir_df_list, &ix->inv_aux,
+                    &ix->mir_dict_list, &ix->mir_df_list, &ix->inv_aux, &ix->inv_fuse,
                     &ix->post_tmp, &ix->lt_keys, &ix->lt_cnt, &ix->lt_g, &ix->lt_pos, &ix->verify_defer, &ix->pairs,
                     &ix->pair_ub, &ix->chunk_list, &ix->chunk_docs, &ix->chunk_fail, &ix->uchunk, &ix->canon_of_slot,
                     &ix->tvals, &ix->term_tmp, &ix->term_esc, &ix->sent_slot, &ix->vcounts, &ix->vnu, &ix->vt_table,
@@ -1370,7 +1373,7 @@
     return TFIDF_OK;
   };
   if (int rc = col_rank()) return rc;
-  HIP_TRY(ix->hctr_h.resize(14));
+  HIP_TRY(ix->hctr_h.resize(14 + 13));
   uint64_t *hctr = ix->hctr_h.data();
   HIP_TRY(hipMemcpyAsync(hctr, ctr, 14 * sizeof(uint64_t), hipMemcpyDeviceToHost, s));
   HIP_TRY(commit_sync(ix, s));
@@ -1539,6 +1542,22 @@
   }
   ix->last_inv_slices = sp.slices;
   ix->last_inv_scan_parts = sp.scan_parts;
+  const bool fused = fuse_plan(S.term_major, S.term_major ? 0u : S.n_blocks - first_block, sp, knob("TFIDF_DF_FROM_ROWS"),
+                               knob("TFIDF_TEST_SCAN_PARTS"), knob("TFIDF_INV_UNFUSED"));
+  ix->last_inv_fused = fused ? 1u : 0u;
+  if (fused) {
+    const uint64_t need = fuse_scratch_words(S.R, S.NC);
+    bool grow = false;
+    const bool zero = fuse_scratch_must_zero(ix->fuse_state, need, &grow);
+    uint64_t words = ix->fuse_state.words;
+    if (grow) {
+      ix->fuse_state = FuseScratch{};
+      HIP_TRY(ix->inv_fuse.reserve((size_t)((need + need / 8 + 4096 + 15) / 16 * 16) * 4));
+      words = ix->inv_fuse.bytes / 4;
+    }
+    if (zero) HIP_TRY(hipMemsetAsync(ix->inv_fuse.p, 0, (size_t)words * 4, s));
+    fuse_scratch_launch(&ix->fuse_state, words);
+  }
   const uint32_t *blk_old = nullptr, *df_old = nullptr;
   if (!S.term_major) {
     const uint64_t blk_need = (uint64_t)(S.n_blocks + 1) * S.NC * 4 + 16;
@@ -1623,6 +1642,8 @@
   pp.df_base = S.df_base.as<uint32_t>();
   pp.df_fold_end = dbp.fold_end;
   pp.df_from_rows = dbp.from_rows ? 1u : 0u;
+  pp.fuse = fused ? ix->inv_fuse.as<uint32_t>() : nullptr;
+  pp.fuse_tickets = fused ? fuse_tickets(sp, N - (uint64_t)first_block * kBlockDocs) : 0u;
   HIP_TRY(hipEventRecord(ix->ev[EV_D0], s));
   if (S.term_major) {
     TermParams tp{};
@@ -1680,14 +1701,16 @@
     HIP_TRY(hipEventRecord(ix->ev[EV_SCAT], s));
   } else {
     if (inv.remap) HIP_TRY(launch_blk_remap(pp, blk_old, df_old, S.crank_inv.as<uint2>(), S.NC_inv, s));
-    if (S.n_blocks) {
+    if (fused) {
+      HIP_TRY(launch_df_fused(pp, s));
+    } else if (S.n_blocks) {
       HIP_TRY(launch_inv_zero(pp, s));
       HIP_TRY(launch_df_partial(pp, s));
     } else {
       HIP_TRY(hipMemsetAsync(S.blk.p, 0, (size_t)S.NC * 4, s));
     }
     HIP_TRY(hipEventRecord(ix->ev[EV_DF], s));
-    HIP_TRY(launch_df_sum(pp, s));
+    if (!fused) HIP_TRY(launch_df_sum(pp, s));
     if (dict_delta || df_delta) {
       MirrorDeltaParams dp{};
       dp.crank = S.crank.as<uint2>();
@@ -1708,9 +1731,9 @@
                               S.sdf.as<uint32_t>(), s));
     }
     if (side_work) HIP_TRY(hipEventRecord(ix->mir_ev[2], s));
-    if (S.n_blocks) HIP_TRY(launch_row_scan(pp, s));
+    if (S.n_blocks && !fused) HIP_TRY(launch_row_scan(pp, s));
     HIP_TRY(hipEventRecord(ix->ev[EV_BSCAN], s));
-    HIP_TRY(launch_block_base(pp, s));
+    if (!fused) HIP_TRY(launch_block_base(pp, s));
     HIP_TRY(hipEventRecord(ix->ev[EV_CSCAN], s));
     if (S.n_blocks) HIP_TRY(launch_scatter(pp, s));
     HIP_TRY(hipEventRecord(ix->ev[EV_SCAT], s));
@@ -1768,8 +1791,8 @@
     if (S.term_major)
       HIP_TRY(launch_count_nonzero(S.dict.as<uint64_t>(), C, reinterpret_cast<unsigned long long *>(ctr + 7), s));
   }
-  uint64_t tail[13];
-  HIP_TRY(hipMemcpyAsync(tail, ctr + 3, sizeof tail, hipMemcpyDeviceToHost, s));
+  uint64_t *tail = hctr + 14;
+  HIP_TRY(hipMemcpyAsync(tail, ctr + 3, 13 * sizeof(uint64_t), hipMemcpyDeviceToHost, s));
   if (!S.term_major) {
     HIP_TRY(S.h_bbase.resize((size_t)S.n_blocks + 2));
     HIP_TRY(hipMemcpyAsync(S.h_bbase.data(), S.bbase.p, ((size_t)S.n_blocks + 1) * 8, hipMemcpyDeviceToHost, s));
@@ -1777,6 +1800,7 @@
   ix->prof.ms_enqueued = prof_ms(ix);
   HIP_TRY(commit_sync(ix, s));
   ix->prof.ms_synced = prof_ms(ix);
+  if (fused) fuse_scratch_done(&ix->fuse_state);
   {
     const EscAppend pe = esc_append_bounds(kept_pe, S.term_major ? 0 : (uint32_t)tail[7], post_esc_cap);
     if (pe.overflow) return fail(TFIDF_E_CAPACITY, "posting escape list overflow");
@@ -1952,6 +1976,13 @@
   std::lock_guard<std::mutex> lk(const_cast<tfidf_index *>(ix)->mu);
   if (slices) *slices = ix->last_inv_slices;
   if (scan_parts) *scan_parts = ix->last_inv_scan_parts;
+  return TFIDF_OK;
+}
+
+extern "C" int tfidf_commit_inversion_fused(const tfidf_index *ix, uint32_t *fused) {
+  if (!ix) return fail(TFIDF_E_INVALID_ARG, "NULL index");
+  std::lock_guard<std::mutex> lk(const_cast<tfidf_index *>(ix)->mu);
+  if (fused) *fused = ix->last_inv_fused;
   return TFIDF_OK;
 }
 
diff --git a/tf-idf-distributed-system_amd/csrc/tfidf_internal.h b/tf-idf-distributed-system_amd/csrc/tfidf_internal.h
--- a/tf-idf-distributed-system_amd/csrc/tfidf_internal.h
+++ b/tf-idf-distributed-system_amd/csrc/tfidf_internal.h
@@ -188,6 +188,8 @@
   uint32_t *df_base;
   uint32_t df_fold_end;
   uint32_t df_from_rows;
+  uint32_t *fuse;
+  uint32_t fuse_tickets;
 };
 
 inline void allow_dyn_lds(const void *fn, int bytes, std::atomic<uint64_t> &done_mask) {
@@ -239,6 +241,7 @@
 hipError_t launch_inv_zero(const PostingParams &p, hipStream_t s);
 hipError_t launch_df_partial(const PostingParams &p, hipStream_t s);
 hipError_t launch_df_sum(const PostingParams &p, hipStream_t s);
+hipError_t launch_df_fused(const PostingParams &p, hipStream_t s);
 hipError_t launch_row_scan(const PostingParams &p, hipStream_t s);
 hipError_t launch_block_base(const PostingParams &p, hipStream_t s);
 hipError_t launch_count_nonzero(const uint64_t *a, uint32_t n, unsigned long long *out, hipStream_t s);
diff --git a/tf-idf-distributed-system_amd/tfidf_amd/_lib.py b/tf-idf-distributed-system_amd/tfidf_amd/_lib.py
--- a/tf-idf-distributed-system_amd/tfidf_amd/_lib.py
+++ b/tf-idf-distributed-system_amd/tfidf_amd/_lib.py
@@ -235,6 +235,7 @@
     "tfidf_commit_tokenized_docs": (C.c_int, [VP, U64P, U32P]),
     "tfidf_commit_inverted_blocks": (C.c_int, [VP, U32P, U32P, U32P]),
     "tfidf_commit_inversion_shape": (C.c_int, [VP, U32P, U32P]),
+    "tfidf_commit_inversion_fused": (C.c_int, [VP, U32P]),
     "tfidf_commit_host_profile": (C.c_int, [VP, C.POINTER(HostProfile)]),
     "tfidf_stats": (C.c_int, [VP, C.POINTER(IndexStats)]),
     "tfidf_search": (C.c_int, [VP, C.c_char_p, C.c_uint64, C.c_uint32, U32P, F32P, C.c_uint64, U64P]),
diff --git a/tf-idf-distributed-system_amd/tfidf_amd/engine.py b/tf-idf-distributed-system_amd/tfidf_amd/engine.py
--- a/tf-idf-distributed-system_amd/tfidf_amd/engine.py
+++ b/tf-idf-distributed-system_amd/tfidf_amd/engine.py
@@ -817,6 +817,11 @@
         L.check(L.load().tfidf_commit_inversion_shape(self._h, C.byref(s), C.byref(p)))
         return {"slices": s.value, "scan_parts": p.value}
 
+    def commit_inversion_fused(self):
+        f = C.c_uint32()
+        L.check(L.load().tfidf_commit_inversion_fused(self._h, C.byref(f)))
+        return bool(f.value)
+
     def commit_host_profile(self):
         p = L.HostProfile()
         L.check(L.load().tfidf_commit_host_profile(self._h, C.byref(p)))
```

New measurement: 9.089 billion, median of 6. +14.2%, better.
